# VitalyVorobyev/calibration

Measured on AMD Instinct MI355X. Metric: residual+Jacobian evals/sec, higher is better.
Workload: dtype f64

## Files before the change

calibration_amd/capi.py:

```python
from __future__ import annotations

import ctypes as C
import os
from typing import Optional

import numpy as np

_HERE = os.path.dirname(os.path.abspath(__file__))

CBA_OK, CBA_ERR_INVALID_ARGUMENT, CBA_ERR_RUNTIME, CBA_ERR_NO_DEVICE, CBA_ERR_HIP, CBA_ERR_INTERNAL = range(6)
CHAIN_INTRINSIC, CHAIN_EXTRINSIC, CHAIN_BUNDLE = 0, 1, 2
HANDEYE_DLT, HANDEYE_GIVEN, HANDEYE_TOO_FEW_VIEWS, HANDEYE_NO_PAIRS, HANDEYE_SINGULAR = range(5)
TARGET_ESTIMATED, TARGET_CONFIG, TARGET_IDENTITY = range(3)
LINEAR_OK, LINEAR_TOO_FEW, LINEAR_DEGENERATE = range(3)
LINEAR_MAX_ITERATIONS = 65536
CAMERA_PINHOLE_BC, CAMERA_SCHEIMPFLUG = 0, 1
DTYPE_U8, DTYPE_F32 = 0, 1
IMAGE_MAX_SIDE = 32768
TRI_OK, TRI_NOT_CONVERGED, TRI_BEHIND, TRI_DEGENERATE, TRI_TOO_FEW = range(5)
TRI_MAX_CAMS = 16
TERM_CONVERGENCE, TERM_NO_CONVERGENCE, TERM_FAILURE = 0, 1, 2
RCCL_UNIQUE_ID_BYTES = 128

c_double_p = C.POINTER(C.c_double)
# ... 187 lines not shown

ALLREDUCE_FN = C.CFUNCTYPE(C.c_int32, c_double_p, C.c_int64, C.c_void_p)


class CbaError(RuntimeError):
    def __init__(self, status: int, message: str):
        super().__init__(f"libcalibba status {status}: {message}")
        self.status = status
        self.message = message


class CbaInvalidArgument(CbaError, ValueError):
    """Maps the reference's std::invalid_argument."""


def dptr(a: Optional[np.ndarray]):
    if a is None:
        return C.cast(None, c_double_p)
    assert a.dtype == np.float64 and a.flags["C_CONTIGUOUS"]
    return a.ctypes.data_as(c_double_p)


def i32ptr(a: Optional[np.ndarray]):
    if a is None:
        return C.cast(None, c_int32_p)
    assert a.dtype == np.int32 and a.flags["C_CONTIGUOUS"]
    return a.ctypes.data_as(c_int32_p)


def u8ptr(a: Optional[np.ndarray]):
    if a is None:
        return C.cast(None, c_uint8_p)
    assert a.dtype == np.uint8 and a.flags["C_CONTIGUOUS"]
    return a.ctypes.data_as(c_uint8_p)


def i64ptr(a: Optional[np.ndarray]):
    if a is None:
        return C.cast(None, c_int64_p)
    assert a.dtype == np.int64 and a.flags["C_CONTIGUOUS"]
    return a.ctypes.data_as(c_int64_p)


def library_path() -> str:
    return os.environ.get("CALIBBA_LIBRARY", os.path.join(_HERE, "lib", "libcalibba.so"))


_LIB = None

PROTOTYPES = {
    "cba_version": (C.c_char_p, []),
    "cba_last_error": (C.c_char_p, []),
    "cba_device_count": (C.c_int32, []),
    "cba_trim_cache": (None, []),
    "cba_set_device": (C.c_int32, [C.c_int32]),
    "cba_get_device": (C.c_int32, []),
    "cba_options_default": (None, [C.POINTER(CbaOptions)]),
    "cba_intrinsics_size": (C.c_int32, [C.c_int32]),
    "cba_local_columns": (C.c_int32, [C.c_int32, C.c_int32]),
    "cba_pose_from_matrix": (None, [c_double_p, c_double_p]),
    "cba_pose_to_matrix": (None, [c_double_p, c_double_p]),
    "cba_reproj_create": (C.c_int32, [C.POINTER(CbaReprojProblem), C.c_int32, C.POINTER(C.c_void_p)]),
    "cba_reproj_create_aos": (C.c_int32, [C.POINTER(CbaReprojProblem), C.POINTER(c_double_p), C.c_int32, C.POINTER(C.c_void_p)]),
    "cba_reproj_destroy": (None, [C.c_void_p]),
    "cba_reproj_set_params": (C.c_int32, [C.c_void_p, c_double_p, c_double_p, c_double_p, c_double_p]),
    "cba_reproj_get_params": (C.c_int32, [C.c_void_p, c_double_p, c_double_p, c_double_p, c_double_p]),
    "cba_reproj_num_observations": (C.c_int64, [C.c_void_p]),
    "cba_reproj_eval": (C.c_int32, [C.c_void_p]),
    "cba_reproj_eval_fetch": (C.c_int32, [C.c_void_p, c_double_p, c_double_p]),
    "cba_reproj_eval_fetch_blocks": (C.c_int32, [C.c_void_p, C.c_int32, C.c_int32, c_double_p, c_double_p]),
    "cba_reproj_eval_timed": (C.c_int32, [C.c_void_p, C.c_int32, C.c_int32, c_double_p]),
    "cba_reproj_normal_eq_timed": (C.c_int32, [C.c_void_p, C.c_int32, C.c_int32, c_double_p]),
    "cba_reproj_set_scalar": (C.c_int32, [C.c_void_p, C.c_int32]),
    "cba_reproj_eval_fetch_f32": (C.c_int32, [C.c_void_p, C.POINTER(C.c_float), C.POINTER(C.c_float)]),
    "cba_reproj_cost": (C.c_int32, [C.c_void_p, C.c_double, c_double_p]),
    "cba_reproj_residual_stats": (C.c_int32, [C.c_void_p, C.c_double, c_double_p, c_double_p]),
    "cba_reproj_residuals_fetch_blocks": (C.c_int32, [C.c_void_p, C.c_int32, C.c_int32, C.c_double, c_double_p, c_uint8_p]),
    "cba_reproj_residual_stats_timed": (C.c_int32, [C.c_void_p, C.c_int32, C.c_int32, c_double_p]),
    "cba_reproj_block_normal_eq": (C.c_int32, [C.c_void_p, c_double_p]),
    "cba_reproj_block_normal_eq_size": (C.c_int64, [C.c_void_p]),
    "cba_reproj_solve": (C.c_int32, [C.c_void_p, C.POINTER(CbaOptions), C.POINTER(CbaSummary)]),
    "cba_reproj_set_lm_mode": (C.c_int32, [C.c_void_p, C.c_int32]),
    "cba_reproj_solve_stats": (C.c_int32, [C.c_void_p, C.POINTER(C.c_int64)]),
    "cba_reproj_covariance_dim": (C.c_int64, [C.c_void_p]),
    "cba_reproj_covariance": (C.c_int32, [C.c_void_p, C.POINTER(CbaOptions), c_double_p]),
    "cba_reproj_covariance_shared_dim": (C.c_int64, [C.c_void_p]),
    "cba_reproj_covariance_shared": (C.c_int32, [C.c_void_p, C.POINTER(CbaOptions), c_double_p]),
    "cba_reproj_covariance_views": (C.c_int32, [C.c_void_p, C.POINTER(CbaOptions), C.c_int32, c_int32_p, c_double_p]),
    "cba_reproj_set_allreduce": (C.c_int32, [C.c_void_p, ALLREDUCE_FN, C.c_void_p, C.c_int32, C.c_int32]),
    "cba_rccl_unique_id": (C.c_int32, [C.POINTER(C.c_uint8)]),
    "cba_reproj_init_rccl": (C.c_int32, [C.c_void_p, C.POINTER(C.c_uint8), C.c_int32, C.c_int32]),
    "cba_optimize_intrinsics": (
        C.c_int32,
        [C.c_int32, C.c_int32, c_int64_p, c_double_p, c_double_p, c_double_p, c_double_p, c_double_p, c_double_p,
         C.POINTER(CbaOptions), C.POINTER(CbaSummary), c_double_p],
    ),
    "cba_optimize_extrinsics": (
        C.c_int32,
        [C.c_int32, C.c_int32, C.c_int32, C.c_int32, c_int64_p, c_int32_p, c_int32_p, c_double_p, c_double_p,
         c_double_p, c_double_p, c_double_p, c_double_p, c_double_p, C.POINTER(CbaOptions), C.POINTER(CbaSummary),
         c_double_p],
    ),
    "cba_optimize_bundle": (
        C.c_int32,
        [C.c_int32, C.c_int32, C.c_int32, c_int64_p, c_int32_p, c_double_p, c_double_p, c_double_p, c_double_p,
         c_double_p, c_double_p, c_double_p, c_double_p, C.POINTER(CbaOptions), C.POINTER(CbaSummary), c_double_p],
    ),
    "cba_optimize_planar_pose": (
        C.c_int32,
        [C.c_int32, c_double_p, c_double_p, c_double_p, c_double_p, c_double_p, C.c_int32, c_double_p, C.POINTER(CbaOptions),
         C.POINTER(CbaSummary), c_double_p, c_double_p, c_double_p],
    ),
    "cba_optimize_planar_pose_batch": (
        C.c_int32,
        [C.c_int32, c_int64_p, c_double_p, c_double_p, c_double_p, c_double_p, c_double_p, C.c_int32, c_double_p,
         C.POINTER(CbaOptions), C.POINTER(CbaSummary), c_double_p, c_double_p, c_double_p],
    ),
    "cba_optimize_homography": (
        C.c_int32,
        [C.c_int32, c_double_p, c_double_p, c_double_p, c_double_p, c_double_p, C.POINTER(CbaOptions), C.POINTER(CbaSummary),
         c_double_p],
    ),
    "cba_optimize_homography_batch": (
        C.c_int32,
        [C.c_int32, c_int64_p, c_double_p, c_double_p, c_double_p, c_double_p, c_double_p, C.POINTER(CbaOptions),
         C.POINTER(CbaSummary), c_double_p],
    ),
    "cba_optimize_intrinsics_semidlt": (
        C.c_int32,
        [C.c_int32, c_int64_p, c_double_p, c_double_p, c_double_p, c_double_p, c_double_p, c_double_p, C.c_int32, c_double_p, c_double_p,
         c_int32_p, c_double_p, C.c_int32, C.POINTER(CbaOptions), C.POINTER(CbaSummary), c_double_p, c_double_p, c_double_p],
    ),
    "cba_optimize_intrinsics_semidlt_sharded": (
        C.c_int32,
        [C.c_int32, c_int64_p, c_double_p, c_double_p, c_double_p, c_double_p, C.c_int32, C.c_int32, c_double_p, c_double_p, C.c_int32,
         c_double_p, c_double_p, c_int32_p, c_double_p, C.c_int32, C.POINTER(CbaOptions), C.POINTER(CbaSummary), c_double_p, c_double_p,
         c_double_p, ALLREDUCE_FN, C.c_void_p, C.c_int32, C.c_int32, C.c_int32],
    ),
    "cba_optimize_intrinsics_semidlt_rccl": (
        C.c_int32,
        [C.c_int32, c_int64_p, c_double_p, c_double_p, c_double_p, c_double_p, C.c_int32, C.c_int32, c_double_p, c_double_p, C.c_int32,
         c_double_p, c_double_p, c_int32_p, c_double_p, C.c_int32, C.POINTER(CbaOptions), C.POINTER(CbaSummary), c_double_p, c_double_p,
         c_double_p, C.POINTER(C.c_uint8), C.c_int32, C.c_int32, C.c_int32],
    ),
    "cba_estimate_homography_batch": (
        C.c_int32, [C.c_int32, c_int64_p, c_double_p, c_double_p, c_double_p, c_double_p, c_double_p, c_int32_p]),
    "cba_estimate_planar_pose_batch": (
        C.c_int32, [C.c_int32, c_int64_p, c_double_p, c_double_p, c_double_p, c_double_p, c_double_p, c_double_p]),
    "cba_estimate_handeye_dlt": (C.c_int32, [C.c_int32, c_double_p, c_double_p, C.c_double, c_double_p]),
    "cba_estimate_and_optimize_handeye": (
        C.c_int32,
        [C.c_int32, c_double_p, c_double_p, C.c_double, c_double_p, C.POINTER(CbaOptions), C.POINTER(CbaSummary), c_double_p],
    ),
    "cba_estimate_and_optimize_handeye_sharded": (
        C.c_int32, [C.c_int32, c_double_p, c_double_p, C.c_double, C.c_int32, c_double_p, C.POINTER(CbaOptions), C.POINTER(CbaSummary),
                    c_double_p, ALLREDUCE_FN, C.c_void_p, C.c_int32, C.c_int32, C.c_int32]),
    "cba_estimate_and_optimize_handeye_rccl": (
        C.c_int32, [C.c_int32, c_double_p, c_double_p, C.c_double, C.c_int32, c_double_p, C.POINTER(CbaOptions), C.POINTER(CbaSummary),
                    c_double_p, C.POINTER(C.c_uint8), C.c_int32, C.c_int32, C.c_int32]),
    "cba_optimize_handeye": (
        C.c_int32,
        [C.c_int32, c_double_p, c_double_p, c_double_p, C.POINTER(CbaOptions), C.POINTER(CbaSummary), c_double_p],
    ),
    "cba_plane_fit_options_default": (None, [C.POINTER(CbaPlaneFitOptions)]),
    "cba_calibrate_laser_plane": (
        C.c_int32,
# ... 134 lines not shown
```

calibration_amd/csrc/backend_hip.hip:

```cpp
#include <rccl/rccl.h>

#include <atomic>
#include <cstring>
#include <mutex>
#include <thread>
#include <set>

#include "engine.hpp"
#include "pipelines.hpp"
#include "lm_core.hpp"
#include "lm_state.hpp"
#include "lm_kernels.hpp"

namespace cba {


static inline unsigned nblk(int64_t n, int per) { return static_cast<unsigned>(std::max<int64_t>(1, (n + per - 1) / per)); }

template <class F>
struct ScopeExit {
    F f;
    ~ScopeExit() { f(); }
};
template <class F>
// ... 49 lines not shown
    template <class F>
    void run_stage(HipLMState::GraphSlot& slot, double huber, bool constrained, F&& enqueue) {
        if (!st.graphs_ok) { enqueue(); return; }
        if (slot.huber != huber || slot.constrained != static_cast<int>(constrained) || slot.scalar != e.scalar) {
            if (slot.exec) (void)hipGraphExecDestroy(slot.exec);
            slot.exec = nullptr;
            slot.uses = 0;
            slot.huber = huber; slot.constrained = static_cast<int>(constrained); slot.scalar = e.scalar;
        }
        if (!slot.exec && slot.uses < st.graph_after) {
            ++slot.uses;
            enqueue();
            return;
        }
        if (!slot.exec) {
            if (hipStreamBeginCapture(e.stream, hipStreamCaptureModeThreadLocal) != hipSuccess) {
                (void)hipGetLastError();
                st.graphs_ok = false;
                enqueue();
                return;
            }
            hipGraph_t graph = nullptr;
            try {
                enqueue();
            } catch (...) {
                (void)hipStreamEndCapture(e.stream, &graph);
                if (graph) (void)hipGraphDestroy(graph);
                throw;
            }
            const hipError_t ec = hipStreamEndCapture(e.stream, &graph);
            const hipError_t ei = (ec == hipSuccess && graph) ? hipGraphInstantiate(&slot.exec, graph, nullptr, nullptr, 0) : hipErrorUnknown;
            if (graph) (void)hipGraphDestroy(graph);
            if (ei != hipSuccess) {
                (void)hipGetLastError();
                slot.exec = nullptr;
                st.graphs_ok = false;
                enqueue();
                return;
            }
        }
        CBA_HIP(hipGraphLaunch(slot.exec, e.stream));
    }

    bool prep_normal_eq(std::vector<double>& cam_acc, double cost2[2]) {
        const Structure& s = st.s;
        cam_acc.assign(static_cast<size_t>(s.n_cams) * s.NACC, 0.0);
        cost2[0] = cost2[1] = 0.0;
        return s.n_blocks != 0;
    }
    void enqueue_normal_eq(double huber, int which = 0, double* cam_out = nullptr, double* cost_out = nullptr) {
        enqueue_normal_eq_head(which, huber);
        enqueue_normal_eq_tail(huber, cam_out, cost_out);
    }
    void enqueue_normal_eq_head(int which, double huber = -1.0, bool consts_done = false) {
        if (!consts_done) launch_block_consts(e, which);
        e.head_huber = st.fuse_small ? huber : -1.0;
        ScopeExit reset{[this] { e.head_huber = -1.0; }};
        launch_normal_eq(e);
    }
    void enqueue_normal_eq_tail(double huber, double* cam_out = nullptr, double* cost_out = nullptr) {
        const Structure& s = st.s;
        const size_t nca = static_cast<size_t>(s.n_cams) * s.NACC;
        if (!cam_out) cam_out = st.pin_ne.p;
        if (!cost_out) cost_out = st.pin_ne.p + nca;
        const bool fused_cost = s.n_blocks <= 4096 && !e.head_weights;
        if (e.head_weights)
            ;
        else if (fused_cost)
            hipLaunchKernelGGL(k_weights_cost, dim3(1), dim3(256), 0, e.stream, s.n_blocks, s.NACC, s.NH + s.PL, e.blk_acc.p, huber,
                               e.blk_w.p, e.blk_s.p, cost_out);
        else
            hipLaunchKernelGGL(k_weights, dim3(nblk(s.n_blocks, 256)), dim3(256), 0, e.stream, s.n_blocks, s.NACC, s.NH + s.PL,
                               e.blk_acc.p, huber, e.blk_w.p, e.blk_s.p);
        hipLaunchKernelGGL(k_cam_partial, dim3(std::max(1, st.n_cchunks)), dim3(256), 0, e.stream, s.NACC, st.cchunk_off.p,
                           st.cam_blk.p, e.blk_w.p, e.blk_acc.p, st.cam_partial.p);
        hipLaunchKernelGGL(k_seg_sum, dim3(nblk(s.NACC, RS_COLS), s.n_cams), dim3(RS_COLS * RS_GROUPS), 0, e.stream, s.n_cams,
                           s.NACC, st.cam_seg.p, st.cam_partial.p, cam_out);
        if (!fused_cost) launch_cost(e, huber, cost_out);
        CBA_HIP(hipGetLastError());
    }
    bool vstats_pending = false;
    double ctl_huber = 0.0;
    bool can_fuse() const { return st.fuse_small && st.schur_wave && st.s.n_views != 0 && !e.scalar; }
    void enqueue_system(double huber, bool tail, bool has_blocks, bool constrained, int which, const PackLayout& L, int has_stats, int has_cost = -1) {
        const Structure& s = st.s;
        const bool q2 = s.n_views != 0;
        if (!can_fuse()) {
            if (tail) enqueue_normal_eq_tail(huber, pack_target() + L.cam, st.stat_dev.p + 4);
            if (q2) enqueue_schur(constrained, which, st.sys_tiles.p);
            enqueue_pack(L, has_blocks, q2, has_stats, has_cost);
            return;
        }
        const int n = s.nsh;
        const int64_t sw = static_cast<int64_t>(st.n_pairs) * 4096;
        if (tail && !e.head_weights)
            hipLaunchKernelGGL(k_weights, dim3(nblk(s.n_blocks, 256)), dim3(256), 0, e.stream, s.n_blocks, s.NACC, s.NH + s.PL, e.blk_acc.p,
                               huber, e.blk_w.p, e.blk_s.p);
        SysArgs a{};
        a.d = st.dims; a.n_views = s.n_views; a.n_blocks = s.n_blocks; a.nsh = n; a.n_tiles = st.n_tiles; a.n_pairs = st.n_pairs;
        a.n_vchunks = st.n_vchunks; a.n_cams = s.n_cams; a.NACC = s.NACC; a.constrained = constrained ? 1 : 0;
        a.n_cc = tail ? std::max(1, st.n_cchunks) : 0;
        a.n_vb = static_cast<int>(nblk(s.n_views, 4));
        a.n_costp = tail ? (s.n_blocks <= 4096 ? 1 : (s.n_blocks + 2047) / 2048) : 0;
        a.n_seg_x = static_cast<int>(nblk(s.NACC, RS_COLS));
        a.n_seg = tail ? a.n_seg_x * s.n_cams : 0;
        a.n_syrk = st.n_vchunks * st.n_pairs;
        a.has_vstats = vstats_pending ? 1 : 0;
        a.huber = huber;
        a.link_off = st.link_off.p; a.cchunk_off = st.cchunk_off.p; a.cam_seg = st.cam_seg.p;
        a.link_blk = st.link_blk.p; a.cam_blk = st.cam_blk.p; a.view_fixed = e.view_fixed.p; a.view_cam_blk = st.view_cam_blk.p;
        a.blk_acc = e.blk_acc.p; a.blk_w = e.blk_w.p; a.blk_s = e.blk_s.p; a.lmp = lmp_src; a.view = e.view[which].p;
        a.view_scale2 = e.view_scale2.p; a.view_L = e.view_L.p; a.view_y = e.view_y.p; a.view_D = e.view_D.p; a.view_gp = e.view_gp.p;
        a.blk_Z = e.blk_Z.p; a.view_gmax = st.view_gmax.p; a.cam_partial = st.cam_partial.p; a.cam_out = pack_target() + L.cam;
        if (a.n_costp > 1) e.cost_part.ensure(static_cast<size_t>(2 * a.n_costp));
        a.cost_part = e.cost_part.p; a.cost_out = st.stat_dev.p + 4;
        a.syrk_partial = st.syrk_partial.p; a.tiles_tail = st.sys_tiles.p + sw + n; a.view_stats = st.view_stats.p; a.stat_out = st.stat_dev.p;
        hipLaunchKernelGGL(k_sys_stage2, dim3(a.n_cc + a.n_vb + a.n_costp), dim3(256), 0, e.stream, a);
        const unsigned g3 = static_cast<unsigned>(a.n_seg + a.n_syrk + 1 + a.has_vstats + (a.n_costp > 1 ? 1 : 0));
        if (n >= 64 && st.syrk_mfma) hipLaunchKernelGGL(k_sys_stage3<true>, dim3(g3), dim3(256), 0, e.stream, a);
        else hipLaunchKernelGGL(k_sys_stage3<false>, dim3(g3), dim3(256), 0, e.stream, a);
        vstats_pending = false;
        hipLaunchKernelGGL(k_sys_pack, dim3(nblk(sw + n, RS_COLS)), dim3(RS_COLS * RS_GROUPS), 0, e.stream,
                           pack_args(L, has_blocks, true, has_stats, has_cost), static_cast<int64_t>(st.n_vchunks), st.syrk_partial.p,
                           st.sys_tiles.p + sw + n, st.stat_dev.p, pack_target());
        CBA_HIP(hipGetLastError());
    }
    void collect_normal_eq(std::vector<double>& cam_acc, double cost2[2]) {
        std::memcpy(cam_acc.data(), st.pin_ne.p, sizeof(double) * cam_acc.size());
        cost2[0] = st.pin_ne.p[cam_acc.size()];
        cost2[1] = st.pin_ne.p[cam_acc.size() + 1];
        e.active = 0;
    }
    bool prep_schur(double radius, bool init_scale, std::vector<double>& S, std::vector<double>& g, double* gmax_priv, int* nfail) {
        const Structure& s = st.s;
        const int n = s.nsh;
        S.assign(static_cast<size_t>(n) * n, 0.0);
        g.assign(n, 0.0);
        *gmax_priv = 0.0;
        *nfail = 0;
        if (s.n_views == 0) return false;
        set_lmp(radius, init_scale);
        return true;
    }
    void enqueue_schur(bool constrained, int which = 0, double* tiles_out = nullptr) {
        const Structure& s = st.s;
        const int n = s.nsh;
        const int vpw = st.schur_wave ? 4 : 64;
        hipLaunchKernelGGL(st.schur_wave ? k_schur_view_wave : k_schur_view, dim3(nblk(s.n_views, vpw)), dim3(st.schur_wave ? 256 : 64), 0,
                           e.stream, st.dims, s.n_views, st.link_off.p, st.link_blk.p, e.blk_acc.p, e.blk_w.p, e.view_fixed.p, lmp_src,
                           constrained ? 1 : 0, e.view[which].p, e.view_scale2.p, e.view_L.p, e.view_y.p, e.view_D.p, e.view_gp.p, e.blk_Z.p,
                           st.view_gmax.p);
        const int64_t sw = static_cast<int64_t>(st.n_pairs) * 4096;
        hipLaunchKernelGGL(n >= 64 && st.syrk_mfma ? k_schur_syrk_mfma : k_schur_syrk, dim3(st.n_vchunks, st.n_pairs), dim3(256), 0, e.stream,
                           st.dims, s.n_views, n, st.n_tiles, st.view_cam_blk.p, e.blk_Z.p, e.view_y.p, st.syrk_partial.p);
        double* pack = tiles_out ? tiles_out : st.pin.p;
        hipLaunchKernelGGL(k_row_sum, dim3(nblk(sw + n, RS_COLS)), dim3(RS_COLS * RS_GROUPS), 0, e.stream, static_cast<int64_t>(st.n_vchunks),
                           sw + n, st.syrk_partial.p, pack);
        hipLaunchKernelGGL(k_col_reduce, dim3(1), dim3(256), 0, e.stream, s.n_views, 0, st.view_gmax.p, st.view_gmax.p, pack + sw + n);
        CBA_HIP(hipGetLastError());
    }
    void collect_schur(std::vector<double>& S, std::vector<double>& g, double* gmax_priv, int* nfail) {
        const Structure& s = st.s;
        const int n = s.nsh;
        const int64_t sw = static_cast<int64_t>(st.n_pairs) * 4096;
        const double* tiles = st.pin.p;
        const int32_t nf = static_cast<int32_t>(tiles[static_cast<size_t>(sw) + n + 1] + 0.5);
        for (int i = 0; i < n; ++i) g[i] = tiles[static_cast<size_t>(sw) + i];
        *gmax_priv = tiles[static_cast<size_t>(sw) + n];
        *nfail = nf;
        int pair = 0;
        for (int ti = 0; ti < st.n_tiles; ++ti)
            for (int tj = ti; tj < st.n_tiles; ++tj, ++pair) {
                const double* T = &tiles[static_cast<size_t>(pair) * 4096];
                for (int a = 0; a < 64; ++a) {
                    const int i = ti * 64 + a;
                    if (i >= n) break;
                    for (int b = 0; b < 64; ++b) {
                        const int j = tj * 64 + b;
                        if (j >= n) break;
                        S[static_cast<size_t>(i) * n + j] = T[a * 64 + b];
                        S[static_cast<size_t>(j) * n + i] = T[a * 64 + b];
                    }
                }
            }
    }

    void normal_eq(double huber, std::vector<double>& cam_acc, double cost2[2]) override {
        if (!prep_normal_eq(cam_acc, cost2)) return;
        enqueue_normal_eq(huber);
        CBA_HIP(hipStreamSynchronize(e.stream));
        collect_normal_eq(cam_acc, cost2);
    }
    void schur(double radius, bool init_scale, bool constrained, std::vector<double>& S, std::vector<double>& g, double* gmax_priv,
               int* nfail) override {
        if (!prep_schur(radius, init_scale, S, g, gmax_priv, nfail)) return;
        run_stage(st.g_schur, 0.0, constrained, [&] { enqueue_schur(constrained); });
        CBA_HIP(hipStreamSynchronize(e.stream));
        collect_schur(S, g, gmax_priv, nfail);
    }
    void normal_eq_schur(double huber, std::vector<double>& cam_acc, double cost2[2], double radius, bool init_scale, bool constrained,
                         std::vector<double>& S, std::vector<double>& g, double* gmax_priv, int* nfail) override {
        const bool q1 = prep_normal_eq(cam_acc, cost2);
        const bool q2 = prep_schur(radius, init_scale, S, g, gmax_priv, nfail);
        if (!q1 && !q2) return;
        run_stage(st.g_new, huber, constrained, [&] {
            if (q1) enqueue_normal_eq(huber);
            if (q2) enqueue_schur(constrained);
        });
        CBA_HIP(hipStreamSynchronize(e.stream));
        if (q1) collect_normal_eq(cam_acc, cost2);
        if (q2) collect_schur(S, g, gmax_priv, nfail);
    }
    PackArgs pack_args(const PackLayout& L, bool has_blocks, bool has_schur, int has_stats, int has_cost) const {
        const Structure& s = st.s;
        PackArgs a;
        a.off_stats = L.stats; a.off_cam = L.cam; a.off_cost = L.cost; a.off_nfail = L.nfail; a.off_S = L.S; a.off_g = L.g; a.off_gmax = L.gmax;
        a.n = s.nsh; a.n_tiles = st.n_tiles; a.n_ranks = L.n_ranks; a.rank = e.rank; a.n_cam_doubles = s.n_cams * s.NACC;
        a.has_blocks = has_blocks; a.has_schur = has_schur; a.has_stats = has_stats; a.has_cost = has_cost < 0 ? has_blocks : has_cost;
        return a;
    }
    void ensure_pack(const PackLayout& L) {
        if (st.pack_dev.n < static_cast<size_t>(L.size)) {
            st.pack_dev.alloc(static_cast<size_t>(L.size));
            st.pack_dev.zero(e.stream);
            st.sys_tiles.alloc(static_cast<size_t>(st.n_pairs) * 4096 + st.s.nsh + 8);
            st.stat_dev.alloc(8);
            st.stat_dev.zero(e.stream);
        }
        st.pin_packed.reserve(static_cast<size_t>(L.size));
    }
    bool host_transport() const { return !e.rccl_comm && e.allreduce != nullptr; }
    double* pack_target() { return host_transport() ? st.pin_packed.p : st.pack_dev.p; }
    void enqueue_pack(const PackLayout& L, bool has_blocks, bool has_schur, int has_stats, int has_cost = -1) {
        const int64_t work = std::max<int64_t>({static_cast<int64_t>(st.s.nsh) * st.s.nsh, static_cast<int64_t>(st.s.n_cams) * st.s.NACC, L.n_ranks, 1});
        hipLaunchKernelGGL(k_pack, dim3(nblk(work, 256)), dim3(256), 0, e.stream, pack_args(L, has_blocks, has_schur, has_stats, has_cost),
                           st.stat_dev.p, st.sys_tiles.p, pack_target());
        CBA_HIP(hipGetLastError());
    }
    void wait_step() {
        if (!st.sync_spin) { CBA_HIP(hipStreamSynchronize(e.stream)); return; }
        if (!st.step_done) CBA_HIP(hipEventCreateWithFlags(&st.step_done, hipEventDisableTiming));
        CBA_HIP(hipEventRecord(st.step_done, e.stream));
        const auto t0 = std::chrono::steady_clock::now();
        for (int spins = 0;; ++spins) {
            const hipError_t q = hipEventQuery(st.step_done);
            if (q == hipSuccess) return;
            if (q != hipErrorNotReady) CBA_HIP(q);
#if defined(__x86_64__)
            __builtin_ia32_pause();
#endif
            if ((spins & 63) == 63 && std::chrono::steady_clock::now() - t0 > std::chrono::microseconds(300)) break;
        }
        CBA_HIP(hipStreamSynchronize(e.stream));
    }
    void exchange(int64_t off, int64_t count, const AllReduce& ar, double* host_out, bool to_device = false) {
        if (e.rccl_comm) {
            const ncclResult_t r = ncclAllReduce(st.pack_dev.p + off, st.pack_dev.p + off, static_cast<size_t>(count), ncclDouble, ncclSum,
                                                 reinterpret_cast<ncclComm_t>(e.rccl_comm), e.stream);
            if (r != ncclSuccess) throw HipError(std::string("ncclAllReduce: ") + ncclGetErrorString(r));
            ++device_allreduce_calls;
            device_allreduce_doubles += count;
        } else if (host_transport()) {
            wait_step();
            ar(st.pin_packed.p + off, count);
            if (to_device) st.pack_dev.upload(st.pin_packed.p + off, static_cast<size_t>(count), e.stream, static_cast<size_t>(off));
            if (host_out) std::memcpy(host_out + off, st.pin_packed.p + off, sizeof(double) * static_cast<size_t>(count));
            return;
        } else {
            ++device_allreduce_calls;
            device_allreduce_doubles += count;
        }
        if (host_out) {
            st.pack_dev.download(st.pin_packed.p + off, static_cast<size_t>(count), e.stream, static_cast<size_t>(off));
            wait_step();
            std::memcpy(host_out + off, st.pin_packed.p + off, sizeof(double) * static_cast<size_t>(count));
        }
    }
    void sys_new(double huber, double radius, bool init_scale, bool constrained, const PackLayout& L, const AllReduce& ar, int rank,
                 double* pack) override {
        (void)rank;
        const Structure& s = st.s;
        ensure_pack(L);
        const bool q1 = s.n_blocks != 0;
        set_lmp(radius, init_scale);
        ctl_huber = huber;
        if (q1) enqueue_normal_eq_head(0, huber);
        enqueue_system(huber, q1, q1, constrained, 0, L, 0);
        exchange(L.cam, L.size - L.cam, ar, pack);
        e.active = 0;
    }
    void sys_resolve(double radius, bool constrained, const PackLayout& L, const AllReduce& ar, int rank, double* pack) override {
        (void)rank;
        const Structure& s = st.s;
        ensure_pack(L);
        set_lmp(radius, false);
        enqueue_system(0.0, false, s.n_blocks != 0, constrained, 0, L, 0, 0);
        exchange(L.nfail, L.gmax - L.nfail, ar, pack);
    }
    bool sys_step(const double* delta_sh, double huber, double radius_next, bool constrained, const PackLayout& L, const AllReduce& ar,
                  int rank, double* pack) override {
        (void)rank;
// ... 19 lines not shown
        const bool q1 = s.n_blocks != 0, q2 = s.n_views != 0;
        e.shared_pack[1].upload(st.pin_pack[1].p, e.pk_delta, e.stream);
        if (q2)
            hipLaunchKernelGGL(k_scale_step, dim3(nblk(s.n_views, 64)), dim3(64), 0, e.stream, s.n_views, a, e.view_fixed.p, e.view[0].p,
                               st.view_delta.p, e.view[1].p, st.view_stats.p);
        if (q1 && want_slope) {
            with_alt_blocks([&] {
                enqueue_normal_eq(huber, 1, pack_target() + L.cam, st.stat_dev.p + 4);
                if (q2)
                    hipLaunchKernelGGL(k_view_slope, dim3(nblk(s.n_views, 64)), dim3(64), 0, e.stream, st.dims, s.n_views, st.link_off.p,
                                       st.link_blk.p, e.blk_acc.p, e.blk_w.p, e.view_fixed.p, st.view_delta.p, st.view_stats.p);
            });
        } else if (q1) {
            launch_block_consts(e, 1);
            launch_resid(e);
            launch_cost(e, huber, st.stat_dev.p + 4);
        }
        if (q2)
            hipLaunchKernelGGL(k_col_reduce, dim3(1), dim3(256), 0, e.stream, s.n_views, 4, st.view_stats.p, static_cast<const double*>(nullptr),
                               st.stat_dev.p);
        else
            CBA_HIP(hipMemsetAsync(st.stat_dev.p, 0, 4 * sizeof(double), e.stream));
        CBA_HIP(hipGetLastError());
        enqueue_pack(L, q1 && want_slope, false, 2, q1 ? 1 : 0);
        exchange(0, L.size, ar, pack);
        e.active = 1;
    }
    void launch_accept() {
        const int64_t n_shared = static_cast<int64_t>(e.pk_delta), n_view = static_cast<int64_t>(e.h_view.size());
        hipLaunchKernelGGL(k_accept, dim3(nblk(std::max(n_shared, n_view), 256)), dim3(256), 0, e.stream, n_shared, e.shared_pack[1].p,
                           e.shared_pack[0].p, n_view, e.view[1].p, e.view[0].p);
    }
    void accept_step() override {
        launch_accept();
        const int64_t n_acc = static_cast<int64_t>(st.s.n_blocks) * st.s.NACC, n_w = st.s.n_blocks;
        if (n_acc > 0)
            hipLaunchKernelGGL(k_accept_blocks, dim3(nblk(n_acc, 256)), dim3(256), 0, e.stream, n_acc, e.blk_acc_alt.p, e.blk_acc.p, n_w,
                               e.blk_w_alt.p, e.blk_w.p);
        CBA_HIP(hipGetLastError());
        e.active = 1;
    }

    bool ctl_constrained = false;
    int64_t ctl_invocations = 0;
    void ensure_ctl(const PackLayout& L) {
        const Structure& s = st.s;
        const int n = s.nsh;
        const int lda = ctl_lda(n), M8 = ctl_padded(n);
        const bool lds = lm_ctl_fits_lds(n);
        const size_t o_scal = 0, o_lmp = CS_COUNT, o_camc = o_lmp + 8, o_gc = o_camc + static_cast<size_t>(s.n_cams) * s.NACC, o_scale2 = o_gc + n,
                     o_hdiag = o_scale2 + n, o_xs = o_hdiag + n, o_rdiag = o_xs + M8, o_xtmp = o_rdiag + M8, o_Ld = o_xtmp + e.pk_size,
                     o_A = o_Ld + static_cast<size_t>(M8) * CTL_NB, total = o_A + (lds ? 8 : static_cast<size_t>(M8 + 1) * lda);
        if (st.ctl_n != n || st.ctl_buf.n < total) {
            st.ctl_buf.alloc(total);
            st.ctl_buf.zero(e.stream);
            st.ctl_idx.alloc(static_cast<size_t>(3 * std::max(1, n)));
            st.ctl_eff.alloc(static_cast<size_t>(std::max(1, n)));
            {
                std::vector<int32_t> tab(static_cast<size_t>(3 * std::max(1, n)), 0);
                CtlView T{};
                T.chain = s.chain; T.PC = s.PC;
                for (int i = 0; i < n; ++i) ctl_decode(T, i, &tab[static_cast<size_t>(n) + i], &tab[static_cast<size_t>(2 * n) + i]);
                st.ctl_idx.upload(tab.data(), tab.size(), e.stream);
                CBA_HIP(hipStreamSynchronize(e.stream));
            }
            st.ctl_rec.reserve(CTL_REC_FETCH + e.pk_size + static_cast<size_t>(n) + 8);
            st.ctl_n = n;
        }
        CtlView& V = st.ctl_view;
        V.n = n; V.n_cams = s.n_cams; V.PI = s.PI; V.PL = s.PL; V.NH = s.NH; V.NACC = s.NACC; V.PC = s.PC; V.sh_base = s.sh_base;
        V.chain = s.chain; V.n_ranks = L.n_ranks;
        V.off_stats = L.stats; V.off_cam = L.cam; V.off_cost = L.cost; V.off_nfail = L.nfail; V.off_S = L.S; V.off_g = L.g; V.off_gmax = L.gmax;
        V.pk_cam = static_cast<int64_t>(e.pk_cam); V.pk_target = static_cast<int64_t>(e.pk_target); V.pk_delta = static_cast<int64_t>(e.pk_delta);
        double* b = st.ctl_buf.p;
        V.x_cur = e.shared_pack[0].p; V.x_trial = e.shared_pack[1].p; V.x_tmp = b + o_xtmp;
        V.scal = b + o_scal; V.lmp = b + o_lmp; V.camc = b + o_camc; V.gc = b + o_gc; V.scale2 = b + o_scale2; V.hdiag = b + o_hdiag; V.xs = b + o_xs;
        V.rdiag = b + o_rdiag; V.A = b + o_A; V.Ld = b + o_Ld; V.lda = lda; V.okflag = nullptr;
        V.pack = st.pack_dev.p;
        V.eff = st.ctl_eff.p; V.idx = st.ctl_idx.p; V.colcam = st.ctl_idx.p + n; V.collc = st.ctl_idx.p + 2 * n;
        V.active = st.res_active.p; V.cam_var = st.res_cam_var.p;
        V.rec = st.ctl_rec.p;
    }
    void run_ctl(int mode, int flag) {
        launch_lm_ctl(st.ctl_view, mode, flag, e.stream);
        ++ctl_invocations;
        if (st.ctl_event) {
            if (!st.ctl_done) CBA_HIP(hipEventCreateWithFlags(&st.ctl_done, hipEventDisableTiming));
            CBA_HIP(hipEventRecord(st.ctl_done, e.stream));
        }
    }
    bool ctl_begin(const CtlSetup& cs, const PackLayout& L) override {
        if (!st.lm_ctl_mode) return false;
        const Structure& s = st.s;
        ensure_pack(L);
        ensure_ctl(L);
        ensure_alt_blocks();
        CtlView& V = st.ctl_view;
        V.eps = cs.eps; V.max_iterations = cs.max_iterations; V.constrained = cs.constrained; V.line_search = cs.line_search;
        V.speculate = (cs.speculate && !e.scalar) ? 1 : 0;
        V.intr_var = cs.intr_var; V.target_var = cs.target_var;
        ctl_constrained = cs.constrained;
        st.pin_mask.reserve(static_cast<size_t>(s.nsh + s.n_cams));
        for (int i = 0; i < s.nsh; ++i) st.pin_mask.p[i] = (*cs.active)[i];
        for (int c = 0; c < s.n_cams; ++c) st.pin_mask.p[s.nsh + c] = (*cs.cam_var)[c];
        st.res_active.upload(st.pin_mask.p, s.nsh, e.stream);
        st.res_cam_var.upload(st.pin_mask.p + s.nsh, s.n_cams, e.stream);
        double* stage = st.ctl_rec.p + CS_COUNT;
        ctl_reset(stage);
        stage[CS_COUNT] = 1e4; stage[CS_COUNT + 1] = 1.0;
        st.ctl_buf.upload(stage, CS_COUNT + 2, e.stream);
        for (int k = 0; k < CS_COUNT; ++k) st.ctl_rec.p[k] = 0.0;
        double* pk = st.pin_pack[0].p;
        stage_shared(pk, cs.intr, cs.cam, cs.target);
        e.shared_pack[0].upload(pk, e.pk_delta, e.stream);
        e.shared_pack[1].upload(pk, e.pk_delta, e.stream);
        lmp_src = V.lmp;
        ctl_invocations = 0;
        st.current_is_on_device = false;
        return true;
    }
    void ctl_new(double huber, bool first, const PackLayout& L, const AllReduce& ar, int rank) override {
        (void)rank;
        const Structure& s = st.s;
        const bool q1 = s.n_blocks != 0;
        ctl_huber = huber;
        if (q1) enqueue_normal_eq_head(0, huber);
        enqueue_system(huber, q1, q1, ctl_constrained, 0, L, 0);
        exchange(L.cam, L.size - L.cam, ar, nullptr, true);
        run_ctl(CTL_NEW, first ? 1 : 0);
        e.active = 0;
    }
    void ctl_resolve(const PackLayout& L, const AllReduce& ar, int rank) override {
        (void)rank;
        const Structure& s = st.s;
        enqueue_system(0.0, false, s.n_blocks != 0, ctl_constrained, 0, L, 0, 0);
        exchange(L.nfail, L.gmax - L.nfail, ar, nullptr, true);
        run_ctl(CTL_RESOLVED, 0);
    }
    void launch_backsub(const double* gate, double* stat_out) {
        const Structure& s = st.s;
        hipLaunchKernelGGL(st.schur_wave ? k_backsub_wave : k_backsub, st.schur_wave ? dim3(nblk(s.n_views, 4)) : dim3(nblk(s.n_views, 64)),
                           st.schur_wave ? dim3(256) : dim3(64), 0, e.stream, st.dims, s.n_views, st.link_off.p, st.link_blk.p, e.d_blk_cam.p,
                           e.blk_Z.p, e.delta_sh.p, e.view_fixed.p, e.view_L.p, e.view_y.p, e.view_D.p, e.view_gp.p, e.view[0].p,
                           st.view_delta.p, e.view[1].p, st.view_stats.p, gate);
        hipLaunchKernelGGL(k_col_reduce, dim3(1), dim3(256), 0, e.stream, s.n_views, 4, st.view_stats.p, static_cast<const double*>(nullptr),
                           stat_out, gate);
    }
    void enqueue_backsub() { launch_backsub(e.gate, st.stat_dev.p); }
    void step_head_speculative() {
        const Structure& s = st.s;
        const bool q1 = s.n_blocks != 0, q2 = s.n_views != 0;
        const bool fused_head = q1 && q2 && can_fuse() && e.chain != CBA_CHAIN_BUNDLE;
        if (fused_head) {
#define CBA_STEP_HEAD(CH)                                                                                                                  \
    hipLaunchKernelGGL(k_step_head<CH>, dim3(nblk(s.n_views, 4)), dim3(256), 0, e.stream, e.gate, st.dims, s.n_views, st.link_off.p,         \
                       st.link_blk.p, e.d_blk_cam.p, e.blk_Z.p, e.delta_sh.p, e.view_fixed.p, e.view_L.p, e.view_y.p, e.view_D.p,          \
                       e.view_gp.p, e.view[0].p, st.view_delta.p, e.view[1].p, st.view_stats.p, e.cam[1].p, e.bc.p)
            if (e.chain == CBA_CHAIN_INTRINSIC) CBA_STEP_HEAD(CH_INTRINSIC); else CBA_STEP_HEAD(CH_EXTRINSIC);
#undef CBA_STEP_HEAD
            launch_camera_consts(e, 1);
            vstats_pending = true;
        } else if (q2) {
            enqueue_backsub();
        } else {
            CBA_HIP(hipMemsetAsync(st.stat_dev.p, 0, 4 * sizeof(double), e.stream));
        }
        if (q1) with_alt_blocks([&] { enqueue_normal_eq_head(1, ctl_huber, fused_head); });
    }
    void step_tail_enqueue(double huber, bool constrained, const PackLayout& L) {
        const Structure& s = st.s;
        const bool q1 = s.n_blocks != 0;
        with_alt_blocks([&] { enqueue_system(huber, q1, q1, constrained, 1, L, 1); });
    }
    void step_tail_speculative(double huber, const PackLayout& L, const AllReduce& ar) {
        step_tail_enqueue(huber, ctl_constrained, L);
        exchange(0, L.size, ar, nullptr, true);
        run_ctl(CTL_STEP, 1);
        e.active = 1;
    }
    void ctl_step(double huber, bool speculative, const PackLayout& L, const AllReduce& ar, int rank) override {
        (void)rank;
        const Structure& s = st.s;
        const bool q1 = s.n_blocks != 0, q2 = s.n_views != 0;
        ctl_huber = huber;
        if (speculative) {
            step_head_speculative();
            step_tail_speculative(huber, L, ar);
            return;
        }
        if (q2) enqueue_backsub();
        else CBA_HIP(hipMemsetAsync(st.stat_dev.p, 0, 4 * sizeof(double), e.stream));
        if (q1) {
            launch_block_consts(e, 1);
            launch_resid(e);
            launch_cost(e, huber, st.stat_dev.p + 4);
        } else {
            CBA_HIP(hipMemsetAsync(st.stat_dev.p + 4, 0, sizeof(double), e.stream));
        }
        enqueue_pack(L, false, false, 1, 1);
        exchange(L.stats, 6, ar, nullptr, true);
        run_ctl(CTL_STEP, 0);
        e.active = 1;
    }
    bool pre_vstats_pending = false, pre_head_weights = false;
    bool ctl_prelaunch() override {
        if (!st.ctl_prelaunch || e.scalar || !e.modeb_shared || (e.chain != CBA_CHAIN_INTRINSIC && !e.modeb_moments)) return false;
        pre_vstats_pending = vstats_pending;
        pre_head_weights = e.head_weights;
        ctl_accept(true);
        e.gate = st.ctl_view.scal + CS_GO;
        bool queued = false;
        ScopeExit reset{[&] {
            e.gate = nullptr;
            if (!queued) ctl_prelaunch_cancel();
        }};
        step_head_speculative();
        queued = true;
        return true;
    }
    void ctl_prelaunch_cancel() override {
        ctl_accept(true);
        vstats_pending = pre_vstats_pending;
        e.head_weights = pre_head_weights;
    }
    void ctl_step_tail(double huber, const PackLayout& L, const AllReduce& ar, int rank) override {
        (void)rank;
        step_tail_speculative(huber, L, ar);
    }
    void ctl_accept(bool blocks) override {
        std::swap(e.view[0].p, e.view[1].p);
        if (blocks) swap_block_sets();
        for (HipLMState::GraphSlot* g : {&st.g_new, &st.g_schur, &st.g_trial})
            if (g->exec) { (void)hipGraphExecDestroy(g->exec); g->exec = nullptr; g->uses = 0; }
    }
    const double* ctl_wait() override {
        volatile const double* seq = st.ctl_rec.p + CS_SEQ;
        const double want = static_cast<double>(ctl_invocations);
        if (st.sync_spin) {
            const auto t0 = std::chrono::steady_clock::now();
            for (int spins = 0; *seq < want; ++spins) {
#if defined(__x86_64__)
                __builtin_ia32_pause();
#endif
                if ((spins & 255) == 255 && std::chrono::steady_clock::now() - t0 > std::chrono::microseconds(st.ctl_poll_us)) break;
            }
        }
        if (*seq < want) {
            const auto t0 = std::chrono::steady_clock::now();
            for (int naps = 0; *seq < want; ++naps) {
                std::this_thread::sleep_for(std::chrono::microseconds(st.ctl_event ? 0 : 30));
                if (st.ctl_event) {
                    CBA_HIP(hipEventSynchronize(st.ctl_done));
                    break;
                }
                if ((naps & 31) != 31) continue;
                const hipError_t q = hipStreamQuery(e.stream);
                if (q == hipSuccess) break;
                if (q != hipErrorNotReady) CBA_HIP(q);
// ... 3 lines not shown
                const bool late = std::chrono::steady_clock::now() - t0 > std::chrono::seconds(st.rccl_timeout_s);
                if (async != ncclSuccess || late) {
                    rccl_abort(e);
                    throw HipError(late ? "RCCL exchange: no progress within the deadline (a peer rank failed or hung); communicator aborted"
                                        : std::string("RCCL exchange failed on a peer: ") + ncclGetErrorString(async) + "; communicator aborted");
                }
            }
            if (*seq < want) throw HipError("LM controller: the control record did not arrive");
        }
        std::atomic_thread_fence(std::memory_order_acquire);
        return st.ctl_rec.p;
    }
    void ctl_fetch(double* intr, double* cam, double* target, double* delta) override {
        double* stage = st.ctl_rec.p + CTL_REC_FETCH;
        e.shared_pack[0].download(stage, e.pk_delta, e.stream);
        e.shared_pack[1].download(stage + e.pk_delta, static_cast<size_t>(st.s.nsh), e.stream, e.pk_delta);
        CBA_HIP(hipStreamSynchronize(e.stream));
        unstage_shared(stage, intr, cam, target);
        std::memcpy(delta, stage + e.pk_delta, sizeof(double) * static_cast<size_t>(st.s.nsh));
    }
    void ctl_line_search_done(const double* scal) override {
        double* stage = st.ctl_rec.p + CS_COUNT;
        std::memcpy(stage, scal, sizeof(double) * CS_COUNT);
        st.ctl_buf.upload(stage, CS_COUNT, e.stream);
        run_ctl(CTL_LS_DONE, 0);
    }

    void trial(const double* delta_sh, double huber, TrialStats* out) override {
        const Structure& s = st.s;
        *out = TrialStats();
        if (s.n_blocks == 0) return;
        std::memcpy(st.pin_pack[1].p + e.pk_delta, delta_sh, sizeof(double) * s.nsh);
        run_stage(st.g_trial, huber, false, [&] {
            e.shared_pack[1].upload(st.pin_pack[1].p, e.pk_delta + static_cast<size_t>(s.nsh), e.stream);
            if (s.n_views > 0) launch_backsub(nullptr, st.pin_tr.p + 8);
            launch_block_consts(e, 1);
            launch_resid(e);
            launch_cost(e, huber, st.pin_tr.p + 24);
            CBA_HIP(hipGetLastError());
        });
        CBA_HIP(hipStreamSynchronize(e.stream));
        e.active = 1;
        const double* h = st.pin_tr.p;
        const double* c2 = st.pin_tr.p + 24;
        out->step2 = s.n_views > 0 ? h[8] : 0.0;
        out->xnorm2 = s.n_views > 0 ? h[9] : 0.0;
        out->gd = s.n_views > 0 ? h[10] : 0.0;
        out->dHd = s.n_views > 0 ? h[11] : 0.0;
        out->cost = c2[0];
    }
    void accept() override {
        launch_accept();
        CBA_HIP(hipGetLastError());
        st.current_is_on_device = true;
    }
    void download_private(double* view_pose) override {
        if (e.h_view.empty()) return;
        e.view[0].download(view_pose, e.h_view.size(), e.stream);
        CBA_HIP(hipStreamSynchronize(e.stream));
    }
    void download_blocks(std::vector<double>& acc, std::vector<double>& w) override {
        acc.resize(static_cast<size_t>(e.n_blocks) * e.NACC);
        w.resize(e.n_blocks);
        e.blk_acc.download(acc.data(), acc.size(), e.stream);
        e.blk_w.download(w.data(), w.size(), e.stream);
        CBA_HIP(hipStreamSynchronize(e.stream));
    }
};

void destroy_lm_state(Engine& e) {
    delete lm_state(e);
    e.lm_state = nullptr;
}

void init_lm_state(Engine& e, const cba_reproj_problem& d, bool have_records) {
    auto* st = new HipLMState();
    e.lm_state = st;
    build_structure(d, st->s, have_records);
    const Structure& s = st->s;
    st->dims = SchurDims{s.PL, s.NH, s.NACC, s.PSH, s.PC, s.n_cams, s.chain};
    st->n_vchunks = std::max(1, (s.n_views + VCHUNK - 1) / VCHUNK);
    st->n_tiles = (s.nsh + 63) / 64;
    st->n_pairs = st->n_tiles * (st->n_tiles + 1) / 2;
    std::vector<int64_t> coff{0}, cseg(s.n_cams + 1, 0);
    for (int c = 0; c < s.n_cams; ++c) {
        for (int64_t p = s.cam_off[c]; p < s.cam_off[c + 1]; p += CCHUNK) coff.push_back(std::min<int64_t>(p + CCHUNK, s.cam_off[c + 1]));
        cseg[c + 1] = static_cast<int64_t>(coff.size()) - 1;
    }
    st->n_cchunks = static_cast<int>(coff.size()) - 1;
    auto up64 = [&](DevBuf<int64_t>& b, const std::vector<int64_t>& v) { b.alloc(v.size()); b.upload(v.data(), v.size(), e.stream); };
    auto up32 = [&](DevBuf<int32_t>& b, const std::vector<int32_t>& v) { b.alloc(v.size()); b.upload(v.data(), v.size(), e.stream); };
    up64(st->cchunk_off, coff);
    up64(st->cam_seg, cseg);
    up32(st->cam_blk, s.cam_blk);
    up64(st->link_off, s.link_off);
    up32(st->link_blk, s.link_blk);
    up32(st->view_cam_blk, s.view_cam_blk);
    st->cam_partial.alloc(static_cast<size_t>(std::max(1, st->n_cchunks)) * s.NACC);
    const size_t nv = std::max(1, s.n_views);
    st->view_gmax.alloc(nv);
    st->view_delta.alloc(nv * 6);
    st->view_delta.zero(e.stream);
    st->view_stats.alloc(nv * 4);
    st->syrk_partial.alloc(static_cast<size_t>(st->n_vchunks) * (static_cast<size_t>(st->n_pairs) * 4096 + s.nsh));
    st->pin.reserve(static_cast<size_t>(st->n_pairs) * 4096 + s.nsh + 8);
    st->pin_ne.reserve(static_cast<size_t>(s.n_cams) * s.NACC + 2);
    st->pin_tr.reserve(32);
    st->pin_lmp.reserve(2);
    st->pin_pack[0].reserve(e.pk_size);
    st->pin_pack[1].reserve(e.pk_size);
    {
        hipFuncAttributes fa;
        (void)hipFuncGetAttributes(&fa, reinterpret_cast<const void*>(k_schur_view));
        warm_reproj_kernels();
    }
    if (const char* env = std::getenv("CBA_SYRK_MFMA")) st->syrk_mfma = std::atoi(env);
    if (const char* env = cba_exp_env("CBA_SCHUR_WAVE")) st->schur_wave = std::atoi(env);
    if (const char* env = cba_exp_env("CBA_LM_FUSE")) st->fuse_small = std::atoi(env);
    if (const char* env = cba_exp_env("CBA_LM_CTL_EVENT")) st->ctl_event = std::atoi(env);
    if (const char* env = cba_exp_env("CBA_SYNC_SPIN")) st->sync_spin = std::atoi(env);
    if (const char* env = std::getenv("CBA_LM_GRAPH")) {
        const int v = std::atoi(env);
        st->graphs_ok = v != 0;
        st->graph_after = v > 1 ? v : (v == 1 ? 0 : st->graph_after);
    }
    e.blk_w.alloc(std::max(1, s.n_blocks));
    e.cam_acc.alloc(static_cast<size_t>(s.n_cams) * s.NACC);
    e.view_L.alloc(nv * 36);
    e.view_y.alloc(nv * 6);
    e.view_D.alloc(nv * 6);
    e.view_gp.alloc(nv * 6);
    e.view_scale2.alloc(nv * 6);
    e.view_fixed.alloc(nv);
    e.view_fixed.zero(e.stream);
    e.blk_Z.alloc(static_cast<size_t>(std::max(1, s.n_blocks)) * 6 * s.PSH);
    e.blk_Z.zero(e.stream);
    up64(st->cam_off, s.cam_off);
    st->res_active.alloc(std::max(1, s.nsh));
    st->res_cam_var.alloc(std::max(1, s.n_cams));
    st->res_Hcc.alloc(static_cast<size_t>(s.nsh) * s.nsh);
    st->res_Ssch.alloc(static_cast<size_t>(s.nsh) * s.nsh);
    st->res_out.alloc(32);
    if (const char* env = cba_exp_env("CBA_LM_CTL")) st->lm_ctl_mode = std::atoi(env) != 0;
    if (const char* env = cba_exp_env("CBA_LM_CTL_POLL_US")) st->ctl_poll_us = std::atoi(env);
    if (const char* env = cba_exp_env("CBA_LM_PRELAUNCH")) st->ctl_prelaunch = std::atoi(env);
    if (const char* env = std::getenv("CBA_RCCL_TIMEOUT_S")) st->rccl_timeout_s = std::max(1, std::atoi(env));
    warm_lm_ctl();
    if (const char* env = std::getenv("CBA_LM_RESIDENT")) st->resident_mode = std::atoi(env);
    if (const char* env = std::getenv("CBA_LM_RESIDENT_MAX_OBS")) st->resident_max_obs = std::atoll(env);
    CBA_HIP(hipStreamSynchronize(e.stream));
}

void solve_stats(const Engine& e, int64_t stats8[8]) {
    const HipLMState* st = reinterpret_cast<const HipLMState*>(e.lm_state);
    for (int k = 0; k < 8; ++k) stats8[k] = st ? st->xs[k] : 0;
}

void set_lm_mode(Engine& e, int mode) {
    if (mode < 0 || mode > 3)
        throw std::invalid_argument("lm mode: 0 chip-wide kernels, 1 automatic, 2 resident kernel whenever possible, 3 chip-wide kernels with the host-side iteration (diagnosis)");
    lm_state(e)->resident_mode = mode == 3 ? 0 : mode;
    lm_state(e)->lm_ctl_mode = mode == 3 ? 0 : 1;
}


static LMDriver make_driver(Engine& e, HipBackend& be) {
    AllReduce ar = [&e](double* buf, int64_t n) { engine_allreduce(e, buf, n); };
    return LMDriver(lm_state(e)->s, be, e.h_intr, e.h_cam, e.h_view, e.h_target, ar, e.n_ranks, e.rank);
}

void warm_lm(Engine& e) {
    cba_options o{};
    o.max_iterations = 1;
    const bool resident = resident_lm_eligible(e, o);
    {
        static std::mutex mu;
        static std::set<uint32_t> warmed;
        const uint32_t key = (static_cast<uint32_t>(e.device) << 8) | (resident ? 0x80u : 0u) | (e.scalar ? 0x40u : 0u) |
                             (static_cast<uint32_t>(e.chain) << 2) | static_cast<uint32_t>(e.model);
        std::lock_guard<std::mutex> lock(mu);
        if (!warmed.insert(key).second) return;
    }
    if (resident) { resident_lm_warm(e); return; }
    HipBackend be(e, *lm_state(e));
    const Structure& s = lm_state(e)->s;
    if (s.n_blocks == 0) return;
    std::vector<double> cam_acc, S, g, d(std::max(1, s.nsh), 0.0);
    double c2[2], gm = 0.0;
    int nf = 0;
    std::vector<int32_t> fixed(s.n_views, 0);
    be.set_view_fixed(fixed);
    be.upload_shared(0, e.h_intr.data(), e.h_cam.data(), e.h_target.data());
    be.normal_eq_schur(1.0, cam_acc, c2, 1e4, true, false, S, g, &gm, &nf);
    std::vector<double> S2, g2;
    be.schur(1e4, false, false, S2, g2, &gm, &nf);
    be.upload_shared(1, e.h_intr.data(), e.h_cam.data(), e.h_target.data());
    TrialStats ts;
    be.trial(d.data(), 1.0, &ts);
    {
        const PackLayout L(s, 1);
        std::vector<double> pack(static_cast<size_t>(L.size), 0.0);
        const AllReduce none = [](double*, int64_t) {};
        void* comm = e.rccl_comm;
        e.rccl_comm = nullptr;
        be.sys_new(1.0, 1e4, true, false, L, none, 0, pack.data());
        be.sys_resolve(1e4, false, L, none, 0, pack.data());
        be.upload_shared(1, e.h_intr.data(), e.h_cam.data(), e.h_target.data());
        (void)be.sys_step(d.data(), 1.0, 1e4, false, L, none, 0, pack.data());
        hipLaunchKernelGGL(k_accept_blocks, dim3(1), dim3(64), 0, e.stream, static_cast<int64_t>(0), e.blk_acc_alt.p, e.blk_acc.p,
                           static_cast<int64_t>(0), e.blk_w_alt.p, e.blk_w.p);
        be.ensure_ctl(L);
        double* stage = lm_state(e)->ctl_rec.p + CS_COUNT;
        ctl_reset(stage);
        stage[CS_TERM] = 0.0;
        lm_state(e)->ctl_buf.upload(stage, CS_COUNT, e.stream);
        be.run_ctl(CTL_NEW, 0);
        e.rccl_comm = comm;
    }
    lm_state(e)->g_new.uses = lm_state(e)->g_schur.uses = lm_state(e)->g_trial.uses = 0;
    CBA_HIP(hipStreamSynchronize(e.stream));
}

void solve_lm(Engine& e, const cba_options& o, cba_summary* out) {
    if (resident_lm_eligible(e, o)) {
        for (int k = 0; k < 8; ++k) lm_state(e)->xs[k] = 0;
        if (resident_lm_solve(e, o, out)) return;
    }
    HipBackend be(e, *lm_state(e));
    LMDriver drv = make_driver(e, be);
    try {
        drv.solve(o, out);
    } catch (...) {
        e.gate = nullptr;
        rccl_abort(e);
        throw;
    }
    {
        const ExchangeStats& x = drv.exchange_stats();
// ... 36 lines not shown
```

calibration_amd/csrc/capi.cpp:

```cpp
#include <algorithm>
#include <chrono>
#include <cmath>
#include <cstdlib>
#include <mutex>
#include <thread>
#include <cstring>
#include <memory>
#include <unordered_map>
#include <vector>

#include "capi_common.hpp"
#include "engine.hpp"
#include "pipelines.hpp"
#include "structure.hpp"

using namespace cba;

__attribute__((visibility("hidden"))) thread_local std::string g_err;
__attribute__((visibility("hidden"))) std::atomic<int> g_default_device{0};

Engine::~Engine() {
    if (stream) (void)hipStreamSynchronize(stream);
    rccl_destroy(*this);
    destroy_lm_state(*this);
// ... 668 lines not shown
    double t = thr * thr;
    for (int i = 0; i < 8 && std::sqrt(t) > thr; ++i) t = std::nextafter(t, 0.0);
    for (int i = 0; i < 8; ++i) {
        const double n = std::nextafter(t, HUGE_VAL);
        if (!(std::sqrt(n) <= thr)) break;
        t = n;
    }
    return t;
}

cba_status cba_reproj_residual_stats(cba_reproj* h, double threshold_px, double* blk_stats, double* total) {
    return guarded([&] {
        require_device();
        Engine& e = *as_engine(h);
        const double t2 = keep_bound(threshold_px);
        CBA_HIP(hipSetDevice(e.device));
        residual_stats(e, t2, blk_stats, total);
    });
}

cba_status cba_reproj_residuals_fetch_blocks(cba_reproj* h, int32_t b0, int32_t b1, double threshold_px, double* r, uint8_t* keep) {
    return guarded([&] {
        require_device();
        Engine& e = *as_engine(h);
        const double t2 = keep_bound(threshold_px);
        if (b0 < 0 || b1 < b0 || b1 > e.n_blocks) throw std::invalid_argument("block range outside the problem");
        CBA_HIP(hipSetDevice(e.device));
        residuals_fetch_range(e, b0, b1, t2, r, keep);
    });
}

cba_status cba_reproj_residual_stats_timed(cba_reproj* h, int32_t fetch, int32_t iters, double* ms) {
    return guarded([&] {
        require_device();
        Engine& e = *as_engine(h);
        if (iters <= 0 || !ms) throw std::invalid_argument("iters must be positive and ms given");
        CBA_HIP(hipSetDevice(e.device));
        for (int i = -1; i < iters; ++i) {
            CBA_HIP(hipEventRecord(e.ev0, e.stream));
            if (fetch) residuals_fetch_range(e, 0, e.n_blocks, HUGE_VAL, nullptr, nullptr);
            else residual_stats_launch(e, HUGE_VAL);
            CBA_HIP(hipEventRecord(e.ev1, e.stream));
            CBA_HIP(hipEventSynchronize(e.ev1));
            float t = 0.f;
            CBA_HIP(hipEventElapsedTime(&t, e.ev0, e.ev1));
            if (i >= 0) ms[i] = static_cast<double>(t);
        }
    });
}

int64_t cba_reproj_block_normal_eq_size(const cba_reproj* h) { return h ? reinterpret_cast<const Engine*>(h)->NACC : 0; }

cba_status cba_reproj_block_normal_eq(cba_reproj* h, double* out) {
    return guarded([&] {
        Engine& e = *as_engine(h);
        CBA_HIP(hipSetDevice(e.device));
        launch_block_consts(e, 0);
        launch_normal_eq(e);
        e.blk_acc.download(out, static_cast<size_t>(e.n_blocks) * e.NACC, e.stream);
        CBA_HIP(hipStreamSynchronize(e.stream));
    });
}

cba_status cba_reproj_solve(cba_reproj* h, const cba_options* opts, cba_summary* summary) {
    return guarded([&] {
        Engine& e = *as_engine(h);
        if (!opts || !summary) throw std::invalid_argument("null argument");
        CBA_HIP(hipSetDevice(e.device));
        solve_lm(e, *opts, summary);
    });
}

cba_status cba_reproj_set_lm_mode(cba_reproj* h, int32_t mode) {
    return guarded([&] { set_lm_mode(*as_engine(h), mode); });
}

cba_status cba_reproj_solve_stats(const cba_reproj* h, int64_t stats8[8]) {
    return guarded([&] {
        if (!h || !stats8) throw std::invalid_argument("null argument");
        solve_stats(*reinterpret_cast<const Engine*>(h), stats8);
    });
}

int64_t cba_reproj_covariance_dim(const cba_reproj* h) { return h ? covariance_dim(*reinterpret_cast<const Engine*>(h)) : 0; }

cba_status cba_reproj_covariance(cba_reproj* h, const cba_options* opts, double* cov) {
    return guarded([&] {
        Engine& e = *as_engine(h);
        if (!opts || !cov) throw std::invalid_argument("null argument");
        CBA_HIP(hipSetDevice(e.device));
        compute_covariance(e, *opts, cov);
    });
}

int64_t cba_reproj_covariance_shared_dim(const cba_reproj* h) { return h ? shared_covariance_dim(*reinterpret_cast<const Engine*>(h)) : 0; }

cba_status cba_reproj_covariance_shared(cba_reproj* h, const cba_options* opts, double* cov) {
    return guarded([&] {
        Engine& e = *as_engine(h);
        if (!opts || !cov) throw std::invalid_argument("null argument");
        CBA_HIP(hipSetDevice(e.device));
        compute_covariance(e, *opts, cov, true);
    });
}

cba_status cba_reproj_covariance_views(cba_reproj* h, const cba_options* opts, int32_t n_sel, const int32_t* view_idx, double* cov7x7) {
    return guarded([&] {
        Engine& e = *as_engine(h);
        if (!opts || n_sel < 0 || (n_sel > 0 && (!view_idx || !cov7x7))) throw std::invalid_argument("null argument");
        if (e.chain == CBA_CHAIN_BUNDLE) throw std::invalid_argument("the bundle chain has no per-view poses");
        CBA_HIP(hipSetDevice(e.device));
        if (n_sel > 0) compute_covariance_views(e, *opts, view_idx, n_sel, cov7x7);
    });
}

cba_status cba_reproj_set_allreduce(cba_reproj* h, cba_allreduce_fn fn, void* user, int32_t n_ranks, int32_t rank) {
    return guarded([&] {
        Engine& e = *as_engine(h);
        if (n_ranks < 1 || rank < 0 || rank >= n_ranks) throw std::invalid_argument("bad rank / n_ranks");
        e.allreduce = fn;
        e.allreduce_user = user;
        e.n_ranks = n_ranks;
        e.rank = rank;
    });
}

cba_status cba_rccl_unique_id(uint8_t id[CBA_RCCL_UNIQUE_ID_BYTES]) {
    return guarded([&] { rccl_unique_id(id); });
}

cba_status cba_reproj_init_rccl(cba_reproj* h, const uint8_t id[CBA_RCCL_UNIQUE_ID_BYTES], int32_t n_ranks, int32_t rank) {
    return guarded([&] {
        Engine& e = *as_engine(h);
        CBA_HIP(hipSetDevice(e.device));
        rccl_init(e, id, n_ranks, rank);
    });
}

static void one_shot(const cba_reproj_problem& d, const cba_options* opts, cba_summary* summary, double* cov) {
    if (!opts || !summary) throw std::invalid_argument("null argument");
    PhaseTimer pt;
    auto e = std::make_unique<Engine>();
    build_engine(d, default_device(), *e);
    pt.lap("one-shot: handle");
    solve_lm(*e, *opts, summary);
    pt.lap("one-shot: solve");
    if (d.intr) std::memcpy(d.intr, e->h_intr.data(), sizeof(double) * e->h_intr.size());
    if (d.cam_pose && d.chain != CBA_CHAIN_INTRINSIC) std::memcpy(d.cam_pose, e->h_cam.data(), sizeof(double) * e->h_cam.size());
    if (d.view_pose && !e->h_view.empty()) std::memcpy(d.view_pose, e->h_view.data(), sizeof(double) * e->h_view.size());
    if (d.target_pose && d.chain == CBA_CHAIN_BUNDLE) std::memcpy(d.target_pose, e->h_target.data(), sizeof(double) * 7);
    if (cov && opts->compute_covariance) {
        try {
            compute_covariance(*e, *opts, cov);
        } catch (const HipError&) {
            throw;
        } catch (const std::runtime_error&) {
            const int64_t n = covariance_dim(*e);
            std::memset(cov, 0, sizeof(double) * static_cast<size_t>(n * n));
        }
    }
    CBA_HIP(hipStreamSynchronize(e->stream));
    pt.lap("one-shot: covariance");
    e.reset();
    pt.lap("one-shot: release");
}

// ... 262 lines not shown
```

calibration_amd/csrc/engine.hpp:

```cpp
#pragma once
#include "hip_glue.hpp"
#include "eval_layout.hpp"

#include <deque>
#include <vector>

#include "../../include/calibba.h"

namespace cba {

struct Tile {
    int32_t blk;
    int32_t count;
    int64_t start;
    int64_t xy_start;
    int64_t reserved;
};

constexpr int OPL_B = 32;
constexpr int TILE_B = 64 * OPL_B;

struct EvalFill {
    bool valid = false;
    int blocked = -1, PL = 0, chain = -1, model = -1;
// ... 20 lines not shown
    int64_t n_tilesA = 0, n_tilesB = 0;
    int32_t max_tileB = 0;

    std::vector<double> h_intr, h_cam, h_view, h_target;

    DevBuf<double> X, Y, u, v, r, J;
    std::deque<DevBuf<double>> Jseg;
    EvalFill J_fill, Jf_fill;
    std::deque<EvalFill> Jseg_fill;
    int64_t seg_tiles = 0;
    double* eval_tile_ptr(int64_t w, int64_t tile_doubles) {
        return Jseg.empty() ? J.p + w * tile_doubles : Jseg[static_cast<size_t>(w / seg_tiles)].p + (w % seg_tiles) * tile_doubles;
    }
    int scalar = 0;
    DevBuf<float> Xf, Yf, uf, vf, Jf, bcf, sdf, intrf;
    DevBuf<double> bc, sd, aux;
    DevBuf<double> shared_pack[2];
    size_t pk_cam = 0, pk_target = 0, pk_delta = 0, pk_size = 0;
    DevBuf<double> intr[2], cam[2], view[2], target[2];
    int eval_blocked = 1;
    int eval_done = 0, eval_blocked_last = 0;
    int eval_ablate = 0;
    int eval_variant = 1;
    int active = 0;
    const double* gate = nullptr;
    double head_huber = -1.0;
    bool head_weights = false;
    DevBuf<int32_t> d_blk_cam, d_blk_view;
    DevBuf<Tile> tilesA, tilesB;
    DevBuf<int64_t> d_blk_tile_off;
    DevBuf<double> partial, blk_acc, blk_s, scalar_out;
    DevBuf<double> diag_part, diag_blk, diag_tot;
    DevBuf<double> diag_fpart, diag_ru, diag_rv;
    DevBuf<uint8_t> diag_keep;
    DevBuf<double> cost_part;
    DevBuf<double> blk_mom;
    int modeb_moments = 1;
    int modeb_shared = 1;
    int modeb_split = -1;

    DevBuf<double> blk_w;
    DevBuf<double> blk_acc_alt, blk_w_alt;
    DevBuf<double> cam_acc;
    DevBuf<double> view_L;
    DevBuf<double> view_y;
    DevBuf<double> view_D;
    DevBuf<double> view_gp;
    DevBuf<double> view_scale2;
    DevBuf<double> blk_Z;
    DevBuf<int32_t> view_fixed;
    DevBuf<double> delta_sh;

    cba_allreduce_fn allreduce = nullptr;
    void* allreduce_user = nullptr;
    void* rccl_comm = nullptr;
    int n_ranks = 1, rank = 0;
    DevBuf<double> coll_buf;
    PinnedBuf<double> coll_pin;
    void* lm_state = nullptr;

    ~Engine();
};

void ensure_f32_buffers(Engine& e);
void launch_block_consts(Engine& e, int which);
void launch_camera_consts(Engine& e, int which);
void launch_eval_fill(Engine& e);
void launch_eval(Engine& e);
void launch_resid(Engine& e);
void warm_reproj_kernels();
void launch_normal_eq(Engine& e);
bool launch_normal_eq_shared_rows(Engine& e, double* rows);
void launch_cost(Engine& e, double huber_delta, double* out = nullptr);

void residual_stats_launch(Engine& e, double t2);
void residual_stats(Engine& e, double t2, double* blk_stats, double* total);
void residuals_fetch_range(Engine& e, int b0, int b1, double t2, double* r, uint8_t* keep);

void init_lm_state(Engine& e, const cba_reproj_problem& d, bool have_records = false);
void destroy_lm_state(Engine& e);
void warm_lm(Engine& e);
void solve_lm(Engine& e, const cba_options& o, cba_summary* out);
void solve_stats(const Engine& e, int64_t stats8[8]);
void set_lm_mode(Engine& e, int mode);
void compute_covariance(Engine& e, const cba_options& o, double* cov, bool shared_only = false);
void compute_covariance_views(Engine& e, const cba_options& o, const int32_t* views, int n_sel, double* view_cov);
int64_t covariance_dim(const Engine& e);
int64_t shared_covariance_dim(const Engine& e);
void engine_allreduce(Engine& e, double* host_buf, int64_t count);
void rccl_unique_id(uint8_t* id);
void rccl_init(Engine& e, const uint8_t* id, int n_ranks, int rank);
void rccl_destroy(Engine& e);
void rccl_abort(Engine& e);

}
```

calibration_amd/csrc/lm_core.hpp:

```cpp
#pragma once
#include <algorithm>
#include <chrono>
#include <cmath>
#include <cstdio>
#include <cstdlib>
#include <cstring>
#include <functional>
#include <limits>
#include <stdexcept>
#include <vector>

#include "dense.hpp"
#include "exp_env.hpp"
#include "line_search.hpp"
#include "lm_ctl.hpp"
#include "reproj_math.hpp"
#include "schur_math.hpp"
#include "structure.hpp"

namespace cba {

struct TrialStats {
    double gd = 0, dHd = 0;
    double step2 = 0, xnorm2 = 0;
// ... 205 lines not shown
        double t_wait = 0, t_queue = 0;
        int n_waits = 0, n_head_queued = 0;
        double rec[CS_COUNT];
        auto wait = [&] {
            const auto a = now();
            const double* r = be_.ctl_wait();
            std::memcpy(rec, r, sizeof(rec));
            t_wait += us(a, now());
            ++n_waits;
        };
        be_.ctl_new(huber, true, L_, ar_, rank_);
        wait();
        double last_printed = 0;
        bool pre = false;
        while (rec[CS_TERM] < 0.0) {
            const auto q0 = now();
            const int expect = static_cast<int>(rec[CS_EXPECT]);
            if (o.verbose && rec[CS_P_ITER] > last_printed) {
                last_printed = rec[CS_P_ITER];
                std::printf("[cba] it %3d cost %.12e cand %.12e rel %.3e radius %.3e |g| %.3e%s\n", static_cast<int>(rec[CS_P_ITER]),
                            rec[CS_P_COST], rec[CS_CAND_COST], rec[CS_REL], rec[CS_P_RADIUS], rec[CS_P_GMAX],
                            rec[CS_SPECULATED] != 0.0 ? " (speculative)" : "");
            }
            bool queued_spec = false;
            if (pre && rec[CS_GO] != 0.0) {
                ++n_head_queued;
                be_.ctl_step_tail(huber, L_, ar_, rank_);
                queued_spec = true;
            } else {
                if (pre) be_.ctl_prelaunch_cancel();
                if (rec[CS_ACCEPT] != 0.0) be_.ctl_accept(rec[CS_ACCEPT] == 2.0);
                if (expect == CTL_STEP) {
                    be_.ctl_step(huber, rec[CS_STEP_SPEC] != 0.0, L_, ar_, rank_);
                    queued_spec = rec[CS_STEP_SPEC] != 0.0;
                } else if (expect == CTL_RESOLVED) {
                    be_.ctl_resolve(L_, ar_, rank_);
                    if (pipeline_ && rec[CS_WILL_END] == 0.0) {
                        be_.ctl_step(huber, rec[CS_STEP_SPEC] != 0.0, L_, ar_, rank_);
                        queued_spec = rec[CS_STEP_SPEC] != 0.0;
                    }
                } else if (expect == CTL_NEW) {
                    be_.ctl_new(huber, false, L_, ar_, rank_);
                } else if (expect == CTL_LINE_SEARCH) {
                    ctl_line_search(huber, rec);
                } else {
                    throw std::runtime_error("LM controller: unexpected request");
                }
            }
            pre = prelaunch_ && queued_spec && be_.ctl_prelaunch();
            t_queue += us(q0, now());
            wait();
        }
        if (pre) be_.ctl_prelaunch_cancel();
        if (rec[CS_ACCEPT] != 0.0) be_.ctl_accept(rec[CS_ACCEPT] == 2.0);
        {
            std::vector<double> d(std::max(1, s_.nsh));
            be_.ctl_fetch(intr_.data(), cam_.data(), target_.data(), d.data());
        }
        if (!view_.empty()) be_.download_private(view_.data());
        xs_.allreduce_calls += be_.device_allreduce_calls;
        xs_.allreduce_doubles += be_.device_allreduce_doubles;
        be_.device_allreduce_calls = be_.device_allreduce_doubles = 0;
        xs_.speculative_steps = static_cast<int32_t>(rec[CS_N_SPEC]);
        xs_.speculation_hits = static_cast<int32_t>(rec[CS_N_HITS]);
        xs_.speculation_misses = static_cast<int32_t>(rec[CS_N_MISSES]);
        xs_.rejected_steps = static_cast<int32_t>(rec[CS_N_REJECTED]);
        cost_ = rec[CS_COST];
        const int term = static_cast<int>(rec[CS_TERM]), iter = static_cast<int>(rec[CS_ITER]);
        out->termination = term;
        out->success = term == CBA_TERM_CONVERGENCE;
        out->iterations = iter;
        out->successful_steps = static_cast<int>(rec[CS_SUCCESSFUL]);
        out->initial_cost = rec[CS_INITIAL_COST];
        out->final_cost = cost_;
        out->solve_seconds = std::chrono::duration<double>(std::chrono::steady_clock::now() - t0).count();
        if (timing)
            std::fprintf(stderr, "[cba timing] solve %.1f us, %d iterations, %d waits: waiting %.1f us, host between a wait and the end of its "
                         "launches %.1f us (%.1f per wait; the host computes nothing there: it reads the record and queues launches), %d of the "
                         "waits returned with the next step's head already queued behind the controller (chip idle for the host: 0), "
                         "controller invocations out of turn %d\n", out->solve_seconds * 1e6, iter, n_waits, t_wait, t_queue,
                         t_queue / std::max(1, n_waits), n_head_queued, static_cast<int>(rec[CS_N_WASTED]));
        if (timing && rec[CS_PROF + CP_PUBLISH] > 0.0) {
            static const char* const names[CTL_NPROF] = {"entry", "adopt", "gradient norm", "assemble", "factorise", "back-substitute", "plus",
                                                         "model terms", "decide", "publish", "", ""};
            std::fprintf(stderr, "[cba timing] controller kernel phases, us over %d invocations:", static_cast<int>(rec[CS_SEQ]));
            for (int k = 0; k <= CP_PUBLISH; ++k) std::fprintf(stderr, " %s %.1f |", names[k], rec[CS_PROF + k] * 0.01);
            std::fprintf(stderr, "\n");
        }
        std::snprintf(out->report, sizeof(out->report), "calibba(schur LM, %d rank%s): %s iters=%d cost %.6e -> %.6e", n_ranks_,
                      n_ranks_ > 1 ? "s" : "", ctl_message(static_cast<int>(rec[CS_MSG])), iter, out->initial_cost, cost_);
        return true;
    }

    void ctl_line_search(double huber, const double* rec) {
        const int n = s_.nsh;
        ++xs_.line_searches;
        std::vector<double> full(n), scaled(n), tintr, tcam, ttarget;
        be_.ctl_fetch(intr_.data(), cam_.data(), target_.data(), full.data());
        const double cost0 = rec[CS_COST], slope0 = rec[CS_SLOPE0], dmax = rec[CS_DMAX];
        double step2_sh = 0, xnorm2_sh = 0;
        auto sample = [&](double a, bool with_slope) {
            for (int i = 0; i < n; ++i) scaled[i] = a * full[i];
            shared_plus(scaled, tintr, tcam, ttarget, &step2_sh, &xnorm2_sh);
            be_.upload_shared(1, tintr.data(), tcam.data(), ttarget.data());
            be_.line_eval(a, huber, with_slope, L_, ar_, rank_, pack_.data());
            LineSample ls;
            ls.step = a;
            ls.value = pack_[L_.stats + PackLayout::TRIAL_COST];
            ls.has_value = std::isfinite(ls.value);
            if (with_slope && ls.has_value) {
                const std::vector<double> cam_acc(pack_.begin() + L_.cam, pack_.begin() + L_.cost);
                std::vector<double> Ht(static_cast<size_t>(n) * n), gt(n);
                assemble_shared(cam_acc, Ht, gt);
                double sl = pack_[L_.stats + PackLayout::SLOPE];
                for (int i = 0; i < n; ++i) sl += gt[i] * full[i];
                ls.slope = sl;
                ls.has_slope = std::isfinite(sl);
            }
            return ls;
        };
        int evals = 0;
        LineSample first;
        first.step = 1.0; first.value = rec[CS_CAND_COST]; first.has_value = std::isfinite(first.value);
        double a = armijo_line_search(cost0, slope0, dmax, sample, &evals, &first);
        xs_.line_search_evaluations += evals;
        if (!(a > 0.0)) {
            a = 1.0;
            (void)sample(1.0, false);
            ++xs_.line_search_evaluations;
        }
        double scal[CS_COUNT];
        std::memcpy(scal, rec, sizeof(scal));
        scal[CS_LS_A] = a;
        scal[CS_LS_COST] = pack_[L_.stats + PackLayout::TRIAL_COST];
        scal[CS_LS_STEP2] = pack_[L_.stats + PackLayout::STEP2];
        scal[CS_LS_XNORM2] = pack_[L_.stats + PackLayout::XNORM2];
        scal[CS_LS_STEP2_SH] = step2_sh;
        scal[CS_LS_XNORM2_SH] = xnorm2_sh;
        scal[CS_EXPECT] = CTL_LS_DONE;
        be_.ctl_line_search_done(scal);
    }

    void solve_host(const cba_options& o, cba_summary* out) {
        const auto t0 = std::chrono::steady_clock::now();
        setup(o);
        const int n = s_.nsh;
        const double eps = o.epsilon, huber = o.huber_delta;
        const double min_radius = 1e-32, max_radius = 1e16, min_rel_decrease = 1e-3;
        double radius = 1e4, decrease_factor = 2.0;
        int iter = 0, invalid = 0, successful = 0;

        project_shared();
        xs_ = ExchangeStats();
        be_.upload_shared(0, intr_.data(), cam_.data(), target_.data());
        new_system(radius, true, huber);
        const double initial_cost = cost_;
        int term = CBA_TERM_FAILURE;
        const char* msg = "";
        std::vector<double> delta(n, 0.0), tintr, tcam, ttarget;
        bool plain_next = false;
        double rel_last = 0.0, rel_prev = 0.0;

        auto done = [&](int t, const char* m) { term = t; msg = m; };
        static const bool timing = [] { const char* e = std::getenv("CBA_LM_TIMING"); return e && e[0] == '1'; }();
        double t_reduced = 0, t_step = 0, t_adopt = 0;
        auto now = [] { return std::chrono::steady_clock::now(); };
        auto us = [](std::chrono::steady_clock::time_point a, std::chrono::steady_clock::time_point b) {
            return std::chrono::duration<double, std::micro>(b - a).count();
        };
// ... 575 lines not shown
```

calibration_amd/csrc/lm_ctl.hip:

```cpp
#include <mutex>
#include <set>

#include "engine.hpp"
#include "lm_ctl.hpp"
#include "lm_state.hpp"
#include "wave_reduce.hpp"

namespace cba {

constexpr int CTL_THREADS = 512;
constexpr int CTL_SMALL_N = 136;
constexpr int CTL_WAVES = CTL_THREADS / 64;

struct BlockTeam {
    double* red;
    double* g_scal;
    unsigned long long* last;
    __device__ __forceinline__ int tid() const { return threadIdx.x; }
    __device__ __forceinline__ int size() const { return CTL_THREADS; }
    __device__ __forceinline__ void sync() const { __syncthreads(); }
    __device__ __forceinline__ double sum(double v) const {
        const double t = wave_sum63(v);
        if ((threadIdx.x & 63) == 63) red[threadIdx.x >> 6] = t;
        __syncthreads();
        double s = 0.0;
#pragma unroll
        for (int w = 0; w < CTL_WAVES; ++w) s += red[w];
        __syncthreads();
        return s;
    }
    __device__ __forceinline__ double max(double v) const {
        for (int o = 32; o > 0; o >>= 1) v = fmax(v, __shfl_xor(v, o));
        if ((threadIdx.x & 63) == 0) red[threadIdx.x >> 6] = v;
        __syncthreads();
        double m = red[0];
#pragma unroll
        for (int w = 1; w < CTL_WAVES; ++w) m = fmax(m, red[w]);
        __syncthreads();
        return m;
    }
    __device__ __forceinline__ int count_before(bool flag, int* total) const {
        const unsigned long long mask = __ballot(flag);
        const int lane = threadIdx.x & 63, wave = threadIdx.x >> 6;
        const int before = __popcll(mask & ((1ull << lane) - 1ull));
        if (lane == 0) red[wave] = static_cast<double>(__popcll(mask));
        __syncthreads();
        int base = 0, tot = 0;
#pragma unroll
        for (int w = 0; w < CTL_WAVES; ++w) {
            const int cw = static_cast<int>(red[w]);
            base += w < wave ? cw : 0;
            tot += cw;
        }
        __syncthreads();
        *total = tot;
        return base + before;
    }
    __device__ __forceinline__ void mark(int) const {}
    __device__ __forceinline__ void tick(const CtlView& V, int slot) const {
        if (threadIdx.x == 0) {
            const unsigned long long t = wall_clock64();
            V.scal[CS_PROF + slot] += static_cast<double>(t - *last);
            *last = t;
        }
    }
    __device__ __forceinline__ void publish(const CtlView& V) const {
        tick(V, CP_PUBLISH);
        __syncthreads();
        const int k = threadIdx.x;
        if (k < CS_COUNT) {
            const double v = V.scal[k];
            g_scal[k] = v;
            if (k != CS_SEQ) V.rec[k] = v;
        }
        __threadfence_system();
        __syncthreads();
        if (k == 0) __hip_atomic_store(&V.rec[CS_SEQ], V.scal[CS_SEQ], __ATOMIC_RELEASE, __HIP_MEMORY_SCOPE_SYSTEM);
    }
};

template <bool LDS_A>
__global__ __launch_bounds__(CTL_THREADS) void k_lm_ctl(CtlView V, int mode, int flag) {
    extern __shared__ double lds_dyn[];
    __shared__ double red[CTL_WAVES];
    __shared__ double s_Ld[LDS_A ? CTL_LDS_MAX_N * CTL_NB : 1];
    __shared__ double s_scal[CS_COUNT];
    __shared__ double s_small[5 * CTL_SMALL_N];
    __shared__ int s_idx[3 * CTL_SMALL_N];
    __shared__ int8_t s_flags[3 * CTL_SMALL_N];
    __shared__ int s_ok;
    __shared__ unsigned long long s_last;
    const int tid = threadIdx.x, n = V.n;
    const bool small = LDS_A || n <= CTL_SMALL_N;
    static_assert(CTL_LDS_MAX_N <= CTL_SMALL_N, "the LDS form keeps the short arrays in LDS too");
    double *g_gc = V.gc, *g_scale2 = V.scale2, *g_hdiag = V.hdiag;
    int* g_idx = V.idx;
    int8_t* g_eff = V.eff;
    if (tid < CS_COUNT) s_scal[tid] = V.scal[tid];
    if (tid == 0) s_last = wall_clock64();
    if (small) {
        for (int i = tid; i < n; i += CTL_THREADS) {
            s_small[2 * CTL_SMALL_N + i] = g_gc[i];
            s_small[3 * CTL_SMALL_N + i] = g_scale2[i];
            s_small[4 * CTL_SMALL_N + i] = g_hdiag[i];
            s_idx[i] = g_idx[i];
            s_idx[CTL_SMALL_N + i] = V.colcam[i];
            s_idx[2 * CTL_SMALL_N + i] = V.collc[i];
            s_flags[i] = g_eff[i];
            s_flags[CTL_SMALL_N + i] = V.active[i];
        }
        for (int c = tid; c < V.n_cams && c < CTL_SMALL_N; c += CTL_THREADS) s_flags[2 * CTL_SMALL_N + c] = V.cam_var[c];
        V.rdiag = s_small; V.xs = s_small + CTL_SMALL_N; V.gc = s_small + 2 * CTL_SMALL_N; V.scale2 = s_small + 3 * CTL_SMALL_N;
        V.hdiag = s_small + 4 * CTL_SMALL_N;
        V.idx = s_idx; V.colcam = s_idx + CTL_SMALL_N; V.collc = s_idx + 2 * CTL_SMALL_N;
        V.eff = s_flags; V.active = s_flags + CTL_SMALL_N;
        if (V.n_cams <= CTL_SMALL_N) V.cam_var = s_flags + 2 * CTL_SMALL_N;
    }
    BlockTeam tm{red, V.scal, &s_last};
    V.scal = s_scal;
    V.okflag = &s_ok;
    if (LDS_A) { V.A = lds_dyn; V.Ld = s_Ld; }
    __syncthreads();
    ctl_run(tm, V, mode, flag);
    if (small)
        for (int i = tid; i < n; i += CTL_THREADS) {
            g_gc[i] = s_small[2 * CTL_SMALL_N + i];
            g_scale2[i] = s_small[3 * CTL_SMALL_N + i];
            g_hdiag[i] = s_small[4 * CTL_SMALL_N + i];
            g_idx[i] = s_idx[i];
            g_eff[i] = s_flags[i];
        }
}

size_t lm_ctl_lds_bytes(int n) { return static_cast<size_t>(ctl_padded(n) + 1) * ctl_lda(n) * sizeof(double); }
bool lm_ctl_fits_lds(int n) { return n <= CTL_LDS_MAX_N; }

void launch_lm_ctl(const CtlView& V, int mode, int flag, hipStream_t stream) {
    if (lm_ctl_fits_lds(V.n))
        hipLaunchKernelGGL(k_lm_ctl<true>, dim3(1), dim3(CTL_THREADS), lm_ctl_lds_bytes(V.n), stream, V, mode, flag);
    else
        hipLaunchKernelGGL(k_lm_ctl<false>, dim3(1), dim3(CTL_THREADS), 0, stream, V, mode, flag);
    CBA_HIP(hipGetLastError());
}

void warm_lm_ctl() {
    static std::mutex mu;
    static std::set<int> done;
    int dev = 0;
    CBA_HIP(hipGetDevice(&dev));
    std::lock_guard<std::mutex> lock(mu);
    if (!done.insert(dev).second) return;
    CBA_HIP(hipFuncSetAttribute(reinterpret_cast<const void*>(k_lm_ctl<true>), hipFuncAttributeMaxDynamicSharedMemorySize,
                                static_cast<int>(lm_ctl_lds_bytes(CTL_LDS_MAX_N))));
    hipFuncAttributes fa;
    (void)hipFuncGetAttributes(&fa, reinterpret_cast<const void*>(k_lm_ctl<false>));
}

}
```

calibration_amd/csrc/lm_ctl.hpp:

```cpp
#pragma once
#include <cmath>
#include <cstdint>

#include "../../include/calibba.h"
#include "reproj_math.hpp"
#include "schur_math.hpp"

#if defined(__HIPCC__)
#define CBA_NOINLINE __host__ __device__ __attribute__((noinline))
#else
#define CBA_NOINLINE inline
#endif

namespace cba {

enum CtlSlot : int {
    CS_SEQ = 0,
    CS_TERM,
    CS_MSG,
    CS_EXPECT,
    CS_STEP_SPEC,
    CS_ACCEPT,
    CS_GO,
    CS_WILL_END,
    CS_RADIUS, CS_DECREASE, CS_RADIUS_SPEC, CS_COST, CS_GMAX, CS_GMAX_PRIV, CS_INITIAL_COST, CS_REL_LAST, CS_REL_PREV,
    CS_ITER, CS_SUCCESSFUL, CS_INVALID, CS_VALID, CS_PLAIN_NEXT, CS_NFAIL, CS_M,
    CS_STEP2_SH, CS_XNORM2_SH, CS_GD_SH, CS_DHD_SH, CS_DMAX,
    CS_CAND_COST, CS_REL, CS_MODEL_CHANGE, CS_SLOPE0, CS_SPECULATED,
    CS_P_COST, CS_P_RADIUS, CS_P_GMAX, CS_P_ITER,
    CS_N_SPEC, CS_N_HITS, CS_N_MISSES, CS_N_REJECTED, CS_N_WASTED,
    CS_LS_A, CS_LS_COST, CS_LS_STEP2, CS_LS_XNORM2, CS_LS_STEP2_SH, CS_LS_XNORM2_SH,
    CS_PROF,
    CS_COUNT = 80
};
constexpr int CTL_NPROF = 12;
enum CtlProf : int { CP_ENTRY = 0, CP_ADOPT, CP_GMAX, CP_ASSEMBLE, CP_FACTOR, CP_BACKSOLVE, CP_PLUS, CP_MODEL, CP_DECIDE, CP_PUBLISH };
static_assert(CS_PROF + CTL_NPROF <= CS_COUNT, "control record size");

enum CtlMode : int { CTL_NONE = 0, CTL_NEW = 1, CTL_RESOLVED = 2, CTL_STEP = 3, CTL_LS_DONE = 4, CTL_LINE_SEARCH = 5 };
enum CtlMsg : int { CM_GRADIENT = 0, CM_MAX_ITER, CM_MIN_RADIUS, CM_INVALID_STEPS, CM_PARAMETER, CM_FUNCTION, CM_NONE };
inline const char* ctl_message(int m) {
    static const char* const k[] = {"Gradient tolerance reached.", "Maximum number of iterations reached.",
                                    "Minimum trust region radius reached.", "Number of consecutive invalid steps more than max.",
                                    "Parameter tolerance reached.", "Function tolerance reached.", ""};
    return k[m < 0 || m > CM_NONE ? CM_NONE : m];
}

constexpr int CTL_NB = 8;
CBA_HD int ctl_padded(int n) { return (n + CTL_NB - 1) / CTL_NB * CTL_NB; }
CBA_HD int ctl_lda(int n) { return ctl_padded(n) | 1; }
constexpr int CTL_LDS_MAX_N = 128;

struct CtlView {
    int n, n_cams, PI, PL, NH, NACC, PC, sh_base, chain, n_ranks;
    int64_t off_stats, off_cam, off_cost, off_nfail, off_S, off_g, off_gmax;
    double eps;
    int max_iterations, constrained, line_search, speculate, intr_var, target_var;
    int64_t pk_cam, pk_target, pk_delta;
    double *x_cur, *x_trial, *x_tmp;
    double* scal;
    const double* pack;
    double* camc;
    double *gc, *scale2, *hdiag;
    const int *colcam, *collc;
    int8_t* eff;
    const int8_t *active, *cam_var;
    int* idx;
    double* A;
    int lda;
    double *rdiag, *xs, *Ld;
    int* okflag;
    double* lmp;
    double* rec;
};

struct SerialTeam {
    CBA_HD int tid() const { return 0; }
    CBA_HD int size() const { return 1; }
    CBA_HD void sync() const {}
    CBA_HD double sum(double v) const { return v; }
    CBA_HD double max(double v) const { return v; }
    CBA_HD int count_before(bool flag, int* total) const { *total = flag ? 1 : 0; return 0; }
    CBA_HD void tick(const CtlView&, int) const {}
    CBA_HD void mark(int) const {}
    CBA_HD void publish(const CtlView& V) const {
        for (int k = 1; k < CS_COUNT; ++k) V.rec[k] = V.scal[k];
        V.rec[CS_SEQ] = V.scal[CS_SEQ];
    }
};

CBA_HD bool ctl_finite(double x) { return fabs(x) <= 1.7976931348623157e308; }

CBA_HD void ctl_decode(const CtlView& V, int i, int* cam, int* lc) {
    if (V.chain == CH_BUNDLE) {
        if (i < 6) { *cam = -1; *lc = i; return; }
        *cam = (i - 6) / V.PC;
        *lc = 6 + (i - 6) - *cam * V.PC;
        return;
    }
    *cam = i / V.PC;
    *lc = 6 + i - *cam * V.PC;
}
template <class VW>
CBA_HD int ctl_intr_base(const VW& V, int c) { return V.chain == CH_INTRINSIC ? 0 : V.sh_base + c * V.PC + 6; }
template <class VW>
CBA_HD int ctl_campose_base(const VW& V, int c) { return V.sh_base + c * V.PC; }
CBA_HD int64_t ctl_sidx(int n, int i, int j) { return i <= j ? static_cast<int64_t>(i) * n - static_cast<int64_t>(i) * (i - 1) / 2 + (j - i)
                                                              : static_cast<int64_t>(j) * n - static_cast<int64_t>(j) * (j - 1) / 2 + (i - j); }

struct CtlPlusView {
    int n_cams, PI, PC, sh_base, chain, intr_var, target_var;
    int64_t pk_cam, pk_target;
    const int8_t* cam_var;
};
struct CtlNorms {
    double step2, xnorm2;
};
CBA_HD CtlPlusView ctl_plus_view(const CtlView& V) {
    return CtlPlusView{V.n_cams, V.PI, V.PC, V.sh_base, V.chain, V.intr_var, V.target_var, V.pk_cam, V.pk_target, V.cam_var};
}
template <class TM>
CBA_NOINLINE CtlNorms ctl_plus(TM tm, CtlPlusView V, const double* x, const double* delta, double* xo) {
    double s2 = 0.0, x2 = 0.0;
    const int PI = V.PI;
    for (int i = tm.tid(); i < V.n_cams * PI; i += tm.size()) {
        const int c = i / PI, k = i - c * PI;
        const double p0 = x[i];
        double p = p0;
        if (V.intr_var) {
            p += delta[ctl_intr_base(V, c) + k];
            if (k < 2) p = fmax(p, 0.0);
            s2 += (p - p0) * (p - p0);
            x2 += p0 * p0;
        }
        xo[i] = p;
    }
    if (V.chain != CH_INTRINSIC)
        for (int c = tm.tid(); c < V.n_cams; c += tm.size()) {
            const double* q = x + V.pk_cam + 7 * c;
            double* o = xo + V.pk_cam + 7 * c;
            for (int k = 0; k < 7; ++k) o[k] = q[k];
            if (V.cam_var[c]) {
                const int pb = ctl_campose_base(V, c);
                quat_plus(q, delta + pb, o);
                for (int k = 0; k < 3; ++k) o[4 + k] = q[4 + k] + delta[pb + 3 + k];
                for (int k = 0; k < 7; ++k) { s2 += (o[k] - q[k]) * (o[k] - q[k]); x2 += q[k] * q[k]; }
            }
        }
    if (V.chain == CH_BUNDLE && tm.tid() == tm.size() - 1) {
        const double* q = x + V.pk_target;
        double* o = xo + V.pk_target;
        for (int k = 0; k < 7; ++k) o[k] = q[k];
        if (V.target_var) {
            quat_plus(q, delta, o);
            for (int k = 0; k < 3; ++k) o[4 + k] = q[4 + k] + delta[3 + k];
            for (int k = 0; k < 7; ++k) { s2 += (o[k] - q[k]) * (o[k] - q[k]); x2 += q[k] * q[k]; }
        }
    }
    CtlNorms r;
    r.step2 = tm.sum(s2);
    r.xnorm2 = tm.sum(x2);
    return r;
}

template <class TM>
CBA_HD double ctl_shared_gmax(TM& tm, const CtlView& V) {
    double m = 0.0;
    if (!V.constrained) {
        for (int i = tm.tid(); i < V.n; i += tm.size())
            if (V.eff[i]) m = fmax(m, fabs(V.gc[i]));
        return tm.max(m);
    }
    if (V.chain == CH_INTRINSIC) {
        if (V.intr_var)
            for (int i = tm.tid(); i < V.n_cams * V.PI; i += tm.size()) {
                const int c = i / V.PI, k = i - c * V.PI, col = ctl_intr_base(V, c) + k;
                const double p0 = V.x_cur[i];
                double p = p0 + (V.eff[col] ? -V.gc[col] : 0.0);
                if (k < 2) p = fmax(p, 0.0);
                m = fmax(m, fabs(p - p0));
            }
        return tm.max(m);
    }
    for (int i = tm.tid(); i < V.n; i += tm.size()) V.xs[i] = V.eff[i] ? -V.gc[i] : 0.0;
    tm.sync();
    (void)ctl_plus(tm, ctl_plus_view(V), V.x_cur, V.xs, V.x_tmp);
    for (int i = tm.tid(); i < V.n_cams * V.PI; i += tm.size()) m = fmax(m, fabs(V.x_tmp[i] - V.x_cur[i]));
    if (V.chain != CH_INTRINSIC)
        for (int i = tm.tid(); i < 7 * V.n_cams; i += tm.size()) m = fmax(m, fabs(V.x_tmp[V.pk_cam + i] - V.x_cur[V.pk_cam + i]));
    if (V.chain == CH_BUNDLE)
        for (int i = tm.tid(); i < 7; i += tm.size()) m = fmax(m, fabs(V.x_tmp[V.pk_target + i] - V.x_cur[V.pk_target + i]));
    return tm.max(m);
// ... 365 lines not shown
        gd += V.gc[i] * di;
    }
    {
        const int PL = V.PL, PL2 = PL * PL;
#pragma unroll 4
        for (int e = tm.tid(); e < V.n_cams * PL2; e += tm.size()) {
            const int c = e / PL2, rem = e - c * PL2, li = rem / PL, lj = rem - li * PL;
            const int gi = ctl_shared_col(V, c, li), gj = ctl_shared_col(V, c, lj);
            if (gi < 0 || gj < 0) continue;
            dHd += delta[gi] * V.camc[static_cast<int64_t>(c) * V.NACC + hidx_sym(PL, li, lj)] * delta[gj];
        }
    }
    gd = tm.sum(gd);
    dHd = tm.sum(dHd);
    dmax = tm.max(dmax);
    tm.tick(V, CP_MODEL);
    if (tm.tid() == 0) {
        V.scal[CS_VALID] = 1.0;
        V.scal[CS_STEP2_SH] = s2; V.scal[CS_XNORM2_SH] = x2; V.scal[CS_GD_SH] = gd; V.scal[CS_DHD_SH] = dHd; V.scal[CS_DMAX] = dmax;
        const double rspec = fmin(CTL_MAX_RADIUS, radius / (1.0 / 3.0));
        V.scal[CS_RADIUS_SPEC] = rspec;
        const bool spec = ctl_next_step_speculative(V);
        V.scal[CS_STEP_SPEC] = spec ? 1.0 : 0.0;
        V.scal[CS_EXPECT] = CTL_STEP;
        V.lmp[0] = spec ? rspec : radius;
        V.lmp[1] = 0.0;
    }
}

template <class TM>
CBA_HD bool ctl_decide(TM& tm, const CtlView& V, bool speculated, double model_change, double cand, double step2, double xnorm2) {
    const double eps = V.eps;
    if (tm.tid() == 0) {
        V.scal[CS_INVALID] = 0.0;
        V.scal[CS_P_COST] = V.scal[CS_COST]; V.scal[CS_P_RADIUS] = V.scal[CS_RADIUS]; V.scal[CS_P_GMAX] = V.scal[CS_GMAX];
        V.scal[CS_P_ITER] = V.scal[CS_ITER];
    }
    if (!ctl_finite(cand)) cand = 1.7976931348623157e308;
    const double cost = V.scal[CS_COST];
    const double step_norm = sqrt(step2), x_norm = sqrt(xnorm2);
    const double cost_change = cost - cand;
    const double rel = cost_change / model_change;
    tm.sync();
    if (tm.tid() == 0) { V.scal[CS_CAND_COST] = cand; V.scal[CS_REL] = rel; V.scal[CS_MODEL_CHANGE] = model_change; V.scal[CS_SPECULATED] = speculated ? 1.0 : 0.0; }
    if (step_norm <= eps * (x_norm + eps)) { ctl_end(tm, V, CBA_TERM_CONVERGENCE, CM_PARAMETER); return false; }
    if (fabs(cost_change) <= eps * cost) { ctl_end(tm, V, CBA_TERM_CONVERGENCE, CM_FUNCTION); return false; }
    if (rel > CTL_MIN_REL_DECREASE) {
        for (int64_t i = tm.tid(); i < V.pk_delta; i += tm.size()) V.x_cur[i] = V.x_trial[i];
        const double radius_old = V.scal[CS_RADIUS];
        const double t3 = 2.0 * rel - 1.0;
        const double radius = fmin(CTL_MAX_RADIUS, radius_old / fmax(1.0 / 3.0, 1.0 - t3 * t3 * t3));
        tm.sync();
        if (tm.tid() == 0) {
            V.scal[CS_SUCCESSFUL] += 1.0;
            V.scal[CS_REL_PREV] = V.scal[CS_REL_LAST];
            V.scal[CS_REL_LAST] = fabs(cost_change) / cost;
            V.scal[CS_RADIUS] = radius;
            V.scal[CS_DECREASE] = 2.0;
            V.scal[CS_PLAIN_NEXT] = 0.0;
            V.scal[CS_ACCEPT] = speculated ? 2.0 : 1.0;
            if (!speculated) {
                V.scal[CS_EXPECT] = CTL_NEW;
                V.lmp[0] = radius;
                V.lmp[1] = 0.0;
            }
        }
        tm.sync();
        return speculated;
    }
    if (tm.tid() == 0) {
        V.scal[CS_N_REJECTED] += 1.0;
        const double radius = V.scal[CS_RADIUS] / V.scal[CS_DECREASE];
        V.scal[CS_RADIUS] = radius;
        V.scal[CS_DECREASE] *= 2.0;
        V.scal[CS_PLAIN_NEXT] = 1.0;
        V.scal[CS_EXPECT] = CTL_RESOLVED;
        V.lmp[0] = radius;
        V.lmp[1] = 0.0;
    }
    return false;
}

template <class TM>
CBA_HD void ctl_run(TM& tm, const CtlView& V, int mode, int flag) {
    const bool in_turn = V.scal[CS_TERM] < 0.0 && static_cast<int>(V.scal[CS_EXPECT]) == mode &&
                         (mode != CTL_STEP || (V.scal[CS_STEP_SPEC] != 0.0) == (flag != 0));
    tm.sync();
    if (tm.tid() == 0) {
        V.scal[CS_SEQ] += 1.0;
        V.scal[CS_GO] = 0.0;
        if (in_turn) { V.scal[CS_ACCEPT] = 0.0; V.scal[CS_WILL_END] = 0.0; }
        else V.scal[CS_N_WASTED] += 1.0;
    }
    tm.sync();
    tm.tick(V, CP_ENTRY);
    enum { AFTER_START = 1, AFTER_NEW = 2, AFTER_STEP = 3 };
    int adopt = 0;
    bool iterate = false;
    if (in_turn) {
        if (mode == CTL_NEW) {
            adopt = flag != 0 ? AFTER_START : AFTER_NEW;
        } else if (mode == CTL_RESOLVED) {
            if (tm.tid() == 0) V.scal[CS_NFAIL] = floor(V.pack[V.off_nfail] + 0.5);
            iterate = true;
        } else {
            const double* st = V.pack + V.off_stats;
            const bool speculated = mode == CTL_STEP && flag != 0;
            const double gd = st[0] + V.scal[CS_GD_SH], dHd = st[1] + V.scal[CS_DHD_SH];
            const double model_change = mode == CTL_STEP ? -gd - 0.5 * dHd : V.scal[CS_MODEL_CHANGE];
            const bool valid = model_change > 0.0 && ctl_finite(model_change);
            double cand = st[4], step2 = st[2] + V.scal[CS_STEP2_SH], xnorm2 = st[3] + V.scal[CS_XNORM2_SH];
            if (mode == CTL_LS_DONE) {
                cand = V.scal[CS_LS_COST];
                step2 = V.scal[CS_LS_STEP2] + V.scal[CS_LS_STEP2_SH];
                xnorm2 = V.scal[CS_LS_XNORM2] + V.scal[CS_LS_XNORM2_SH];
            }
            tm.sync();
            if (tm.tid() == 0 && speculated) V.scal[CS_N_SPEC] += 1.0;
            if (!valid) {
                ctl_invalid_step(tm, V);
            } else if (mode == CTL_STEP && V.constrained && V.line_search && !(ctl_finite(cand) && cand <= V.scal[CS_COST] + 1e-4 * gd)) {
                if (tm.tid() == 0) {
                    V.scal[CS_MODEL_CHANGE] = model_change;
                    V.scal[CS_SLOPE0] = gd;
                    V.scal[CS_CAND_COST] = cand;
                    V.scal[CS_EXPECT] = CTL_LINE_SEARCH;
                }
            } else if (ctl_decide(tm, V, speculated, model_change, cand, step2, xnorm2)) {
                adopt = AFTER_STEP;
            }
        }
        tm.sync();
        tm.tick(V, CP_DECIDE);
    }
    if (adopt) {
        ctl_adopt(tm, V, adopt == AFTER_START);
        if (adopt == AFTER_START) {
            if (tm.tid() == 0) V.scal[CS_INITIAL_COST] = V.scal[CS_COST];
            if (V.scal[CS_GMAX] <= V.eps) ctl_end(tm, V, CBA_TERM_CONVERGENCE, CM_GRADIENT);
            else iterate = true;
        } else if (adopt == AFTER_NEW) {
            iterate = true;
        } else if (V.scal[CS_RADIUS] != V.scal[CS_RADIUS_SPEC]) {
            if (tm.tid() == 0) {
                V.scal[CS_N_MISSES] += 1.0;
                V.scal[CS_EXPECT] = CTL_RESOLVED;
                V.lmp[0] = V.scal[CS_RADIUS];
                V.lmp[1] = 0.0;
            }
        } else {
            if (tm.tid() == 0) V.scal[CS_N_HITS] += 1.0;
            iterate = true;
        }
        tm.sync();
    }
    if (iterate) ctl_iterate(tm, V);
    tm.sync();
    if (tm.tid() == 0 && static_cast<int>(V.scal[CS_EXPECT]) == CTL_RESOLVED && V.scal[CS_TERM] < 0.0) {
        int term, msg;
        V.scal[CS_WILL_END] = ctl_top_tests(V, &term, &msg) ? 1.0 : 0.0;
        V.scal[CS_STEP_SPEC] = ctl_next_step_speculative(V) ? 1.0 : 0.0;
    }
    if (tm.tid() == 0)
        V.scal[CS_GO] = (in_turn && V.scal[CS_TERM] < 0.0 && static_cast<int>(V.scal[CS_EXPECT]) == CTL_STEP && V.scal[CS_STEP_SPEC] != 0.0 &&
                         V.scal[CS_ACCEPT] == 2.0) ? 1.0 : 0.0;
    tm.sync();
    tm.publish(V);
// ... 13 lines not shown
```

calibration_amd/csrc/lm_kernels.hpp:

```cpp
#pragma once
#include "block_reduce.hpp"
#include "lm_ctl.hpp"
#include "schur_math.hpp"
#include "wave_reduce.hpp"

namespace cba {

constexpr int VCHUNK = 8;
constexpr size_t CTL_REC_FETCH = 2 * CS_COUNT + 8;
constexpr int CCHUNK = 16;

__global__ void k_weights(int n_blocks, int NACC, int s_idx, const double* __restrict__ blk_acc, double huber_delta,
                          double* __restrict__ blk_w, double* __restrict__ blk_s) {
    const int b = blockIdx.x * blockDim.x + threadIdx.x;
    if (b >= n_blocks) return;
    const double s = blk_acc[static_cast<int64_t>(b) * NACC + s_idx];
    double rho, w;
    huber(s, huber_delta, &rho, &w);
    blk_w[b] = w;
    blk_s[b] = s;
}

__global__ __launch_bounds__(256) void k_weights_cost(int n_blocks, int NACC, int s_idx, const double* __restrict__ blk_acc,
                                                      double huber_delta, double* __restrict__ blk_w, double* __restrict__ blk_s,
                                                      double* __restrict__ out) {
    __shared__ double sh[2][256];
    double c = 0.0, ss = 0.0;
    constexpr int NQ = 16;
    for (int b0 = static_cast<int>(threadIdx.x); b0 < n_blocks; b0 += NQ * 256) {
        double sv[NQ];
#pragma unroll
        for (int q = 0; q < NQ; ++q) {
            const int b = b0 + q * 256;
            sv[q] = b < n_blocks ? blk_acc[static_cast<int64_t>(b) * NACC + s_idx] : 0.0;
        }
#pragma unroll
        for (int q = 0; q < NQ; ++q) {
            const int b = b0 + q * 256;
            if (b < n_blocks) {
                double rho, w;
                huber(sv[q], huber_delta, &rho, &w);
                blk_w[b] = w;
                blk_s[b] = sv[q];
                c += 0.5 * rho;
                ss += sv[q];
            }
        }
    }
    block_sum2(sh, c, ss, out);
}

__device__ __forceinline__ void cam_partial_body(int k, int NACC, const int64_t* __restrict__ chunk_off, const int32_t* __restrict__ cam_blk,
                                                 const double* __restrict__ blk_w, const double* __restrict__ blk_acc,
                                                 double* __restrict__ partial) {
    const int64_t p0 = chunk_off[k], p1 = chunk_off[k + 1];
    for (int e = threadIdx.x; e < NACC; e += blockDim.x) {
        double s = 0.0;
        for (int64_t p = p0; p < p1; p += CCHUNK) {
            double a[CCHUNK], w[CCHUNK];
#pragma unroll
            for (int q = 0; q < CCHUNK; ++q) {
                const bool in = p + q < p1;
                const int b = in ? cam_blk[p + q] : 0;
                w[q] = in ? blk_w[b] : 0.0;
                a[q] = in ? blk_acc[static_cast<int64_t>(b) * NACC + e] : 0.0;
            }
#pragma unroll
            for (int q = 0; q < CCHUNK; ++q)
                if (p + q < p1) s += w[q] * a[q];
        }
        partial[static_cast<int64_t>(k) * NACC + e] = s;
    }
}
__global__ void k_cam_partial(int NACC, const int64_t* __restrict__ chunk_off, const int32_t* __restrict__ cam_blk,
                              const double* __restrict__ blk_w, const double* __restrict__ blk_acc,
                              double* __restrict__ partial) {
    cam_partial_body(blockIdx.x, NACC, chunk_off, cam_blk, blk_w, blk_acc, partial);
}

constexpr int RS_COLS = 32, RS_GROUPS = 8;

__device__ __forceinline__ double grouped_column_sum(const double* __restrict__ rows, int64_t t0, int64_t t1, int64_t width,
                                                     int64_t e, bool valid, double (*sh)[RS_COLS]) {
    const int c = threadIdx.x % RS_COLS, r = threadIdx.x / RS_COLS;
    double s = 0.0;
    if (valid)
// ... 198 lines not shown
    const int c = threadIdx.x;
    if (c >= 64 || c0 + c >= nsh) return;
    double s = 0.0;
    for (int r = 0; r < nrow; ++r) s += Zs[r][c] * ysh[r];
    out[c0 + c] = s;
}

constexpr int SYRK_ROWS = 6 * VCHUNK;
constexpr int SYRK_LDS = 2 * SYRK_ROWS * 64 + SYRK_ROWS + VCHUNK * SYRK_MAX_CAMS / 2;

__device__ __forceinline__ void tile_pair(int pair, int n_tiles, int* ti, int* tj) {
    int i = 0;
    while (pair >= n_tiles - i) { pair -= n_tiles - i; ++i; }
    *ti = i;
    *tj = i + pair;
}

__device__ __forceinline__ void syrk_tile_valu(const double (*Zi)[64], const double (*Zc)[64], int nrow, double* __restrict__ out) {
    const int tx = threadIdx.x & 15, ty = threadIdx.x >> 4;
    double acc[4][4];
#pragma unroll
    for (int a = 0; a < 4; ++a)
#pragma unroll
        for (int b = 0; b < 4; ++b) acc[a][b] = 0.0;
    for (int r = 0; r < nrow; ++r) {
        double a[4], b[4];
#pragma unroll
        for (int q = 0; q < 4; ++q) { a[q] = Zi[r][ty * 4 + q]; b[q] = Zc[r][tx * 4 + q]; }
#pragma unroll
        for (int p = 0; p < 4; ++p)
#pragma unroll
            for (int q = 0; q < 4; ++q) acc[p][q] += a[p] * b[q];
    }
#pragma unroll
    for (int p = 0; p < 4; ++p)
#pragma unroll
        for (int q = 0; q < 4; ++q) out[(ty * 4 + p) * 64 + tx * 4 + q] = acc[p][q];
}

typedef double v4f64 __attribute__((ext_vector_type(4)));
__device__ __forceinline__ void syrk_tile_mfma(const double (*Zi)[64], const double (*Zc)[64], double* __restrict__ out) {
    const int lane = threadIdx.x & 63, wave = threadIdx.x >> 6;
    const int li = lane & 15, lk = lane >> 4;
    v4f64 acc[4];
#pragma unroll
    for (int c = 0; c < 4; ++c) acc[c] = v4f64{0.0, 0.0, 0.0, 0.0};
#pragma unroll
    for (int step = 0; step < SYRK_ROWS / 4; ++step) {
        const int r = 4 * step + lk;
        const double a = Zi[r][wave * 16 + li];
#pragma unroll
        for (int c = 0; c < 4; ++c) acc[c] = __builtin_amdgcn_mfma_f64_16x16x4f64(a, Zc[r][c * 16 + li], acc[c], 0, 0, 0);
    }
#pragma unroll
    for (int c = 0; c < 4; ++c)
#pragma unroll
        for (int reg = 0; reg < 4; ++reg) out[(wave * 16 + lk + 4 * reg) * 64 + c * 16 + li] = acc[c][reg];
}

template <bool MFMA>
__device__ __forceinline__ void schur_syrk_body(double* lds, int bx, int by, int gy, const SchurDims& d, int n_views, int nsh, int n_tiles,
        const int32_t* __restrict__ view_cam_blk, const double* __restrict__ blk_Z, const double* __restrict__ y, double* __restrict__ partial) {
    double (*Zi)[64] = reinterpret_cast<double (*)[64]>(lds), (*Zj)[64] = Zi + SYRK_ROWS;
    double* ysh = lds + 2 * SYRK_ROWS * 64;
    int* bsh = reinterpret_cast<int*>(ysh + SYRK_ROWS);
    int ti, tj;
    tile_pair(by, n_tiles, &ti, &tj);
    const int i0 = ti * 64, j0 = tj * 64;
    const int v0 = bx * VCHUNK;
    const int nrow = 6 * (min(n_views, v0 + VCHUNK) - v0);
    stage_block_table(d, n_views, v0, view_cam_blk, bsh);
    __syncthreads();
    stage_Z(d, bsh, n_views, v0, view_cam_blk, blk_Z, i0, nsh, Zi);
    if (tj != ti) stage_Z(d, bsh, n_views, v0, view_cam_blk, blk_Z, j0, nsh, Zj);
    if (static_cast<int>(threadIdx.x) < SYRK_ROWS) ysh[threadIdx.x] = static_cast<int>(threadIdx.x) < nrow ? y[6 * static_cast<int64_t>(v0) + threadIdx.x] : 0.0;
    __syncthreads();
    const double (*Zc)[64] = tj != ti ? Zj : Zi;
    double* row = partial + static_cast<int64_t>(bx) * (static_cast<int64_t>(gy) * 4096 + nsh);
    double* out = row + static_cast<int64_t>(by) * 4096;
    if constexpr (MFMA) syrk_tile_mfma(Zi, Zc, out);
    else syrk_tile_valu(Zi, Zc, nrow, out);
    if (ti == tj) schur_gvec_chunk(Zi, ysh, nrow, i0, nsh, row + static_cast<int64_t>(gy) * 4096);
}
__global__ __launch_bounds__(256) void k_schur_syrk(SchurDims d, int n_views, int nsh, int n_tiles, const int32_t* __restrict__ view_cam_blk,
        const double* __restrict__ blk_Z, const double* __restrict__ y, double* __restrict__ partial) {
    __shared__ double lds[SYRK_LDS];
    schur_syrk_body<false>(lds, blockIdx.x, blockIdx.y, gridDim.y, d, n_views, nsh, n_tiles, view_cam_blk, blk_Z, y, partial);
}
__global__ __launch_bounds__(256) void k_schur_syrk_mfma(SchurDims d, int n_views, int nsh, int n_tiles, const int32_t* __restrict__ view_cam_blk,
        const double* __restrict__ blk_Z, const double* __restrict__ y, double* __restrict__ partial) {
    __shared__ double lds[SYRK_LDS];
    schur_syrk_body<true>(lds, blockIdx.x, blockIdx.y, gridDim.y, d, n_views, nsh, n_tiles, view_cam_blk, blk_Z, y, partial);
}

__global__ void k_backsub(SchurDims d, int n_views, const int64_t* __restrict__ link_off, const int32_t* __restrict__ link_blk,
                          const int32_t* __restrict__ blk_cam, const double* __restrict__ blk_Z,
                          const double* __restrict__ delta_sh, const int32_t* __restrict__ fixed, const double* __restrict__ L,
                          const double* __restrict__ y, const double* __restrict__ D, const double* __restrict__ gp,
                          const double* __restrict__ x, double* __restrict__ delta_p, double* __restrict__ xt,
                          double* __restrict__ stats , const double* __restrict__ gate = nullptr) {
    if (gate && *gate == 0.0) return;
    const int v = blockIdx.x * blockDim.x + threadIdx.x;
    if (v >= n_views) return;
    const int nb = static_cast<int>(link_off[v + 1] - link_off[v]);
    double o4[4];
    backsub_view_body(d, nb, link_blk + link_off[v], blk_cam, blk_Z, delta_sh, fixed[v] != 0, L + 36 * static_cast<int64_t>(v),
                      y + 6 * static_cast<int64_t>(v), D + 6 * static_cast<int64_t>(v), gp + 6 * static_cast<int64_t>(v),
                      x + 7 * static_cast<int64_t>(v), delta_p + 6 * static_cast<int64_t>(v), xt + 7 * static_cast<int64_t>(v), o4);
    for (int k = 0; k < 4; ++k) stats[4 * static_cast<int64_t>(v) + k] = o4[k];
}

__global__ void k_accept(int64_t n_shared, const double* __restrict__ shared_trial, double* __restrict__ shared_cur, int64_t n_view,
                         const double* __restrict__ view_trial, double* __restrict__ view_cur) {
    const int64_t i = static_cast<int64_t>(blockIdx.x) * blockDim.x + threadIdx.x;
    if (i < n_shared) shared_cur[i] = shared_trial[i];
    if (i < n_view) view_cur[i] = view_trial[i];
}

struct PackArgs {
    int64_t off_stats, off_cam, off_cost, off_nfail, off_S, off_g, off_gmax;
    int n, n_tiles, n_ranks, rank, n_cam_doubles;
    int has_blocks , has_cost , has_schur, has_stats;
};
__device__ __forceinline__ void pack_scalars(const PackArgs& a, const double* __restrict__ stat, double nfail, double* __restrict__ pack) {
    pack[a.off_nfail] = nfail;
    pack[a.off_cost] = a.has_cost ? stat[4] : 0.0;
    pack[a.off_stats + 0] = a.has_stats == 1 ? stat[2] : 0.0;
    pack[a.off_stats + 1] = a.has_stats == 1 ? stat[3] : 0.0;
    pack[a.off_stats + 2] = a.has_stats ? stat[0] : 0.0;
    pack[a.off_stats + 3] = a.has_stats ? stat[1] : 0.0;
    pack[a.off_stats + 4] = (a.has_stats && a.has_cost) ? stat[4] : 0.0;
    pack[a.off_stats + 5] = a.has_stats == 2 ? stat[2] : 0.0;
}
__global__ __launch_bounds__(256) void k_pack(PackArgs a, const double* __restrict__ stat ,
                                              const double* __restrict__ tiles , double* __restrict__ pack) {
    const int64_t tid = static_cast<int64_t>(blockIdx.x) * blockDim.x + threadIdx.x;
    const int64_t nn = static_cast<int64_t>(a.n) * a.n;
    const int64_t sw = static_cast<int64_t>(a.n_tiles) * (a.n_tiles + 1) / 2 * 4096;
    if (tid < nn) {
        const int i = static_cast<int>(tid / a.n), j = static_cast<int>(tid % a.n);
        if (i <= j) {
            double val = 0.0;
            if (a.has_schur) {
                const int ti = i >> 6, tj = j >> 6;
                const int pair = ti * a.n_tiles - ti * (ti - 1) / 2 + (tj - ti);
                val = tiles[static_cast<int64_t>(pair) * 4096 + (i & 63) * 64 + (j & 63)];
            }
            pack[a.off_S + ctl_sidx(a.n, i, j)] = val;
        }
    }
    if (tid < a.n) pack[a.off_g + tid] = a.has_schur ? tiles[sw + tid] : 0.0;
    if (tid < a.n_ranks) pack[a.off_gmax + tid] = (a.has_schur && tid == a.rank) ? tiles[sw + a.n] : 0.0;
    if (tid == 0) pack_scalars(a, stat, a.has_schur ? tiles[sw + a.n + 1] : 0.0, pack);
    if (!a.has_blocks && tid < a.n_cam_doubles) pack[a.off_cam + tid] = 0.0;
}

struct SysArgs {
    SchurDims d;
    int n_views, n_blocks, nsh, n_tiles, n_pairs, n_vchunks, n_cams, NACC, constrained;
    int n_cc, n_vb, n_costp;
    int n_seg_x, n_seg, n_syrk;
    int has_vstats;
    double huber;
    const int64_t *link_off, *cchunk_off, *cam_seg;
    const int32_t *link_blk, *cam_blk, *view_fixed, *view_cam_blk;
    const double *blk_acc, *blk_w, *blk_s, *lmp, *view;
    double *view_scale2, *view_L, *view_y, *view_D, *view_gp, *blk_Z, *view_gmax, *cam_partial, *cam_out, *cost_part, *cost_out;
    double *syrk_partial, *tiles_tail , *view_stats, *stat_out;
};

__global__ __launch_bounds__(256) void k_sys_stage2(SysArgs a) {
    __shared__ double lds[2 * 256];
    int bx = blockIdx.x;
    if (bx < a.n_cc) {
        cam_partial_body(bx, a.NACC, a.cchunk_off, a.cam_blk, a.blk_w, a.blk_acc, a.cam_partial);
        return;
    }
    bx -= a.n_cc;
    if (bx < a.n_vb) {
        schur_view_wave_body(bx, a.d, a.n_views, a.link_off, a.link_blk, a.blk_acc, a.blk_w, a.view_fixed, a.lmp, a.constrained, a.view,
                             a.view_scale2, a.view_L, a.view_y, a.view_D, a.view_gp, a.blk_Z, a.view_gmax);
        return;
    }
    bx -= a.n_vb;
    if (a.n_costp == 1) cost_range_body(lds, 0, a.n_blocks, a.blk_s, a.huber, a.cost_out);
    else cost_range_body(lds, bx * 2048, min(bx * 2048 + 2048, a.n_blocks), a.blk_s, a.huber, a.cost_part + 2 * bx);
}

template <bool MFMA>
__global__ __launch_bounds__(256) void k_sys_stage3(SysArgs a) {
    __shared__ double lds[SYRK_LDS];
    static_assert(SYRK_LDS >= COL_REDUCE_LDS && SYRK_LDS >= RS_GROUPS * RS_COLS, "one LDS buffer for every body");
    int bx = blockIdx.x;
    if (bx < a.n_seg) {
        seg_sum_body(lds, bx % a.n_seg_x, bx / a.n_seg_x, a.NACC, a.cam_seg, a.cam_partial, a.cam_out);
        return;
    }
    bx -= a.n_seg;
    if (bx < a.n_syrk) {
        const int chunk = bx % a.n_vchunks, pair = bx / a.n_vchunks;
        schur_syrk_body<MFMA>(lds, chunk, pair, a.n_pairs, a.d, a.n_views, a.nsh, a.n_tiles, a.view_cam_blk, a.blk_Z, a.view_y, a.syrk_partial);
        return;
    }
    bx -= a.n_syrk;
    if (bx == 0) { col_reduce_body(lds, a.n_views, 0, a.view_gmax, a.view_gmax, a.tiles_tail); return; }
    if (bx == 1 && a.has_vstats) { col_reduce_body(lds, a.n_views, 4, a.view_stats, nullptr, a.stat_out); return; }
    if (threadIdx.x == 0) {
        double c = 0.0, ss = 0.0;
        for (int k = 0; k < a.n_costp; ++k) { c += a.cost_part[2 * k]; ss += a.cost_part[2 * k + 1]; }
        a.cost_out[0] = c;
        a.cost_out[1] = ss;
    }
}

__global__ __launch_bounds__(RS_COLS * RS_GROUPS) void k_sys_pack(PackArgs a, int64_t n_rows, const double* __restrict__ rows,
                                                                   const double* __restrict__ tail ,
                                                                   const double* __restrict__ stat, double* __restrict__ pack) {
    __shared__ double sh[RS_GROUPS][RS_COLS];
    const int64_t sw = static_cast<int64_t>(a.n_tiles) * (a.n_tiles + 1) / 2 * 4096, width = sw + a.n;
    const int64_t e = static_cast<int64_t>(blockIdx.x) * RS_COLS + threadIdx.x % RS_COLS;
    const double tot = grouped_column_sum(rows, 0, n_rows, width, e, e < width, sh);
    if (threadIdx.x < RS_COLS && e < width) {
        if (e < sw) {
            int ti, tj;
            tile_pair(static_cast<int>(e >> 12), a.n_tiles, &ti, &tj);
            const int i = ti * 64 + static_cast<int>((e >> 6) & 63), j = tj * 64 + static_cast<int>(e & 63);
            if (i <= j && j < a.n) pack[a.off_S + ctl_sidx(a.n, i, j)] = tot;
        } else {
            pack[a.off_g + (e - sw)] = tot;
        }
    }
    const int64_t tid = static_cast<int64_t>(blockIdx.x) * blockDim.x + threadIdx.x;
    if (tid < a.n_ranks) pack[a.off_gmax + tid] = tid == a.rank ? tail[0] : 0.0;
    if (tid == 0) pack_scalars(a, stat, tail[1], pack);
    if (!a.has_blocks)
        for (int64_t k = tid; k < a.n_cam_doubles; k += static_cast<int64_t>(gridDim.x) * blockDim.x) pack[a.off_cam + k] = 0.0;
}

template <int CHAIN>
__global__ __launch_bounds__(256) void k_step_head(const double* __restrict__ gate, SchurDims d, int n_views, const int64_t* __restrict__ link_off,
                                                   const int32_t* __restrict__ link_blk, const int32_t* __restrict__ blk_cam,
                                                   const double* __restrict__ blk_Z, const double* __restrict__ delta_sh,
                                                   const int32_t* __restrict__ fixed, const double* __restrict__ L, const double* __restrict__ y,
                                                   const double* __restrict__ D, const double* __restrict__ gp, const double* __restrict__ x,
                                                   double* __restrict__ delta_p, double* __restrict__ xt, double* __restrict__ stats,
                                                   const double* __restrict__ cam_trial, double* __restrict__ bc) {
    if (gate && *gate == 0.0) return;
    const int v = blockIdx.x * 4 + (threadIdx.x >> 6), lane = threadIdx.x & 63;
    if (v >= n_views) return;
    const int nb = static_cast<int>(link_off[v + 1] - link_off[v]);
    const int32_t* blks = link_blk + link_off[v];
    const bool fx = fixed[v] != 0;
    double a[6];
    backsub_wave_sums(d, nb, blks, blk_cam, blk_Z, delta_sh, fx, lane, a);
    double pose[7] = {0.0, 0.0, 0.0, 0.0, 0.0, 0.0, 0.0};
    if (lane == 63) {
        double o4[4], dp[6];
        backsub_view_finish(fx, a, L + 36 * static_cast<int64_t>(v), y + 6 * static_cast<int64_t>(v), D + 6 * static_cast<int64_t>(v),
                            gp + 6 * static_cast<int64_t>(v), x + 7 * static_cast<int64_t>(v), dp, pose, o4);
        for (int k = 0; k < 6; ++k) delta_p[6 * static_cast<int64_t>(v) + k] = dp[k];
        for (int k = 0; k < 7; ++k) xt[7 * static_cast<int64_t>(v) + k] = pose[k];
        for (int k = 0; k < 4; ++k) stats[4 * static_cast<int64_t>(v) + k] = o4[k];
    }
#pragma unroll
    for (int k = 0; k < 7; ++k) pose[k] = __shfl(pose[k], 63);
    for (int k = lane; k < nb; k += 64) {
        const int b = blks[k];
        double out[BC_SIZE];
        block_consts<CHAIN>(pose, CHAIN == CH_EXTRINSIC ? cam_trial + 7 * static_cast<int64_t>(blk_cam[b]) : nullptr, nullptr, out);
        for (int i = 0; i < BC_SIZE; ++i) bc[static_cast<int64_t>(b) * BC_SIZE + i] = out[i];
    }
}

__global__ void k_scale_step(int n_views, double a, const int32_t* __restrict__ fixed, const double* __restrict__ x,
                             const double* __restrict__ delta_p, double* __restrict__ xt, double* __restrict__ stats) {
    const int v = blockIdx.x * blockDim.x + threadIdx.x;
    if (v >= n_views) return;
    double o2[2];
    scale_step_view_body(fixed[v] != 0, a, x + 7 * static_cast<int64_t>(v), delta_p + 6 * static_cast<int64_t>(v), xt + 7 * static_cast<int64_t>(v), o2);
    stats[4 * static_cast<int64_t>(v)] = o2[0];
    stats[4 * static_cast<int64_t>(v) + 1] = o2[1];
    stats[4 * static_cast<int64_t>(v) + 2] = 0.0;
    stats[4 * static_cast<int64_t>(v) + 3] = 0.0;
}
__global__ void k_view_slope(SchurDims d, int n_views, const int64_t* __restrict__ link_off, const int32_t* __restrict__ link_blk,
                             const double* __restrict__ blk_acc, const double* __restrict__ blk_w, const int32_t* __restrict__ fixed,
                             const double* __restrict__ delta_p, double* __restrict__ stats) {
    const int v = blockIdx.x * blockDim.x + threadIdx.x;
    if (v >= n_views) return;
    stats[4 * static_cast<int64_t>(v) + 2] = view_slope_body(d, static_cast<int>(link_off[v + 1] - link_off[v]), link_blk + link_off[v], blk_acc,
                                                              blk_w, fixed[v] != 0, delta_p + 6 * static_cast<int64_t>(v));
}

__global__ void k_accept_blocks(int64_t n_acc, const double* __restrict__ acc_trial, double* __restrict__ acc_cur, int64_t n_w,
                                const double* __restrict__ w_trial, double* __restrict__ w_cur) {
    const int64_t i = static_cast<int64_t>(blockIdx.x) * blockDim.x + threadIdx.x;
    if (i < n_acc) acc_cur[i] = acc_trial[i];
    if (i < n_w) w_cur[i] = w_trial[i];
}

}
```

calibration_amd/csrc/lm_state.hpp:

```cpp
#pragma once
#include "engine.hpp"
#include "lm_ctl.hpp"
#include "schur_math.hpp"
#include "structure.hpp"

namespace cba {

struct HipLMState {
    Structure s;
    SchurDims dims;
    int n_vchunks = 0, n_tiles = 0, n_pairs = 0, n_cchunks = 0;
    int fuse_small = 1;
    int schur_wave = 1;
    int syrk_mfma = 1;
    DevBuf<int32_t> view_cam_blk, cam_blk;
    DevBuf<int64_t> cchunk_off, cam_seg, link_off;
    DevBuf<int32_t> link_blk;
    DevBuf<double> cam_partial, view_gmax, view_delta, view_stats, syrk_partial;
    PinnedBuf<double> pin, pin_ne, pin_tr;
    DevBuf<double> pack_dev, sys_tiles, stat_dev;
    PinnedBuf<double> pin_packed;
    hipEvent_t step_done = nullptr;
    hipEvent_t ctl_done = nullptr;
    int ctl_event = 0;
    int sync_spin = 1;
    ~HipLMState() {
        if (step_done) (void)hipEventDestroy(step_done);
        if (ctl_done) (void)hipEventDestroy(ctl_done);
    }
    int64_t xs[8] = {0, 0, 0, 0, 0, 0, 0, 0};
    struct GraphSlot {
        hipGraphExec_t exec = nullptr;
        double huber = 0.0;
        int constrained = -1, scalar = -1;
        int uses = 0;
        ~GraphSlot() { if (exec) (void)hipGraphExecDestroy(exec); }
    };
    GraphSlot g_new, g_schur, g_trial;
    bool graphs_ok = true;
    int graph_after = 200;
    PinnedBuf<double> pin_lmp;
    PinnedBuf<double> pin_pack[2];
    bool current_is_on_device = false;
    int resident_mode = 1;
    int64_t resident_max_obs = -1;
    DevBuf<int64_t> cam_off;
    DevBuf<int8_t> res_active, res_cam_var;
    DevBuf<double> res_Hcc, res_Ssch, res_out;
    PinnedBuf<double> pin_res;
    PinnedBuf<int8_t> pin_mask;
    DevBuf<double> ctl_buf;
    DevBuf<int32_t> ctl_idx;
    DevBuf<int8_t> ctl_eff;
    PinnedBuf<double> ctl_rec;
    CtlView ctl_view{};
    int ctl_n = -1;
    int rccl_timeout_s = 120;
    int ctl_prelaunch = 1;
    int ctl_poll_us = 2000;
    int lm_ctl_mode = 1;
};


inline HipLMState* lm_state(Engine& e) { return reinterpret_cast<HipLMState*>(e.lm_state); }

bool resident_lm_eligible(const Engine& e, const cba_options& o);
void resident_lm_warm(Engine& e);
bool resident_lm_solve(Engine& e, const cba_options& o, cba_summary* out, bool keep_parameters = false);

void launch_lm_ctl(const CtlView& V, int mode, int flag, hipStream_t stream);
bool lm_ctl_fits_lds(int n);
void warm_lm_ctl();

}
```

calibration_amd/optim.py:

```python
from __future__ import annotations

import ctypes as C
from dataclasses import dataclass, field
from typing import List, Optional, Sequence

import numpy as np

from . import capi
from .capi import CbaOptions, CbaReprojProblem, CbaSummary, dptr, i32ptr, i64ptr


@dataclass
class OptimOptions:
    optimizer: int = 0
    huber_delta: float = 1.0
    epsilon: float = 1e-9
    max_iterations: int = 1000
    compute_covariance: bool = True
    verbose: bool = False


@dataclass
class OptimResult:
    success: bool = False
# ... 287 lines not shown
                getattr(f, name)[...] = np.asarray(val, dtype=np.float64).reshape(getattr(f, name).shape)
        capi.check(self.lib, self.lib.cba_reproj_set_params(self.h, dptr(f.intr), dptr(f.cam_pose), dptr(f.view_pose),
                                                            dptr(f.target_pose)))

    def get_params(self):
        f = self.flat
        capi.check(self.lib, self.lib.cba_reproj_get_params(self.h, dptr(f.intr), dptr(f.cam_pose), dptr(f.view_pose),
                                                            dptr(f.target_pose)))
        return f.intr, f.cam_pose, f.view_pose, f.target_pose

    def eval(self):
        capi.check(self.lib, self.lib.cba_reproj_eval(self.h))

    def eval_fetch(self):
        n, p = self.n_obs, self.local_columns
        r = np.zeros(2 * n)
        J = np.zeros((2 * n, p))
        capi.check(self.lib, self.lib.cba_reproj_eval_fetch(self.h, dptr(r), dptr(J)))
        return r, J

    def eval_fetch_blocks(self, b0: int, b1: int):
        n, p = int(self.flat.blk_offset[b1] - self.flat.blk_offset[b0]), self.local_columns
        r = np.zeros(2 * n)
        J = np.zeros((2 * n, p))
        capi.check(self.lib, self.lib.cba_reproj_eval_fetch_blocks(self.h, int(b0), int(b1), dptr(r), dptr(J)))
        return r, J

    def set_scalar(self, scalar: int):
        capi.check(self.lib, self.lib.cba_reproj_set_scalar(self.h, int(scalar)))

    def eval_fetch_f32(self):
        n, p = self.n_obs, self.local_columns
        r = np.zeros(2 * n, dtype=np.float32)
        J = np.zeros((2 * n, p), dtype=np.float32)
        capi.check(self.lib, self.lib.cba_reproj_eval_fetch_f32(self.h, r.ctypes.data_as(C.POINTER(C.c_float)),
                                                                J.ctypes.data_as(C.POINTER(C.c_float))))
        return r, J

    def eval_timed(self, warmup: int, iters: int) -> float:
        ms = C.c_double(0.0)
        capi.check(self.lib, self.lib.cba_reproj_eval_timed(self.h, int(warmup), int(iters), C.byref(ms)))
        return float(ms.value)

    def normal_eq_timed(self, warmup: int, iters: int) -> float:
        ms = C.c_double()
        capi.check(self.lib, self.lib.cba_reproj_normal_eq_timed(self.h, int(warmup), int(iters), C.byref(ms)))
        return ms.value

    def cost(self, huber_delta: float = 1.0) -> float:
        c = C.c_double(0.0)
        capi.check(self.lib, self.lib.cba_reproj_cost(self.h, float(huber_delta), C.byref(c)))
        return float(c.value)

    def residual_stats(self, threshold_px: float = float("inf")):
        from .diagnostics import ResidualStats

        nb = self.flat.n_blocks
        blk = np.zeros((max(nb, 1), 4))
        tot = np.zeros(4)
        capi.check(self.lib, self.lib.cba_reproj_residual_stats(self.h, float(threshold_px), dptr(blk), dptr(tot)))
        return ResidualStats.from_flat(self.flat, blk[:nb], tot, float(threshold_px))

    def residuals_fetch_blocks(self, b0: int, b1: int, threshold_px: float = float("inf")):
        n = int(self.flat.blk_offset[b1] - self.flat.blk_offset[b0]) if 0 <= b0 <= b1 <= self.flat.n_blocks else 0
        r = np.zeros(max(2 * n, 1))
        keep = np.zeros(max(n, 1), dtype=np.uint8)
        capi.check(self.lib, self.lib.cba_reproj_residuals_fetch_blocks(self.h, int(b0), int(b1), float(threshold_px), dptr(r),
                                                                        capi.u8ptr(keep)))
        return r[:2 * n], keep[:n].astype(bool)

    def residual_stats_timed(self, iters: int = 5, fetch: bool = False) -> np.ndarray:
        ms = np.zeros(int(iters))
        capi.check(self.lib, self.lib.cba_reproj_residual_stats_timed(self.h, int(bool(fetch)), int(iters), dptr(ms)))
        return ms

    def block_normal_eq(self) -> np.ndarray:
        w = int(self.lib.cba_reproj_block_normal_eq_size(self.h))
        out = np.zeros((self.flat.n_blocks, w))
        capi.check(self.lib, self.lib.cba_reproj_block_normal_eq(self.h, dptr(out)))
        return out

    def set_lm_mode(self, mode: int):
        capi.check(self.lib, self.lib.cba_reproj_set_lm_mode(self.h, int(mode)))

    def solve_stats(self) -> dict:
        a = (C.c_int64 * 8)()
        capi.check(self.lib, self.lib.cba_reproj_solve_stats(self.h, a))
        return dict(zip(("allreduce_calls", "allreduce_doubles", "speculative_steps", "speculation_hits", "speculation_misses",
                         "rejected_steps", "line_searches", "line_search_evaluations"), (int(v) for v in a)))

    def solve(self, opts: CbaOptions) -> CbaSummary:
        s = CbaSummary()
        capi.check(self.lib, self.lib.cba_reproj_solve(self.h, C.byref(opts), C.byref(s)))
        self.get_params()
        return s

    def covariance(self, opts: CbaOptions) -> Optional[np.ndarray]:
        dim = int(self.lib.cba_reproj_covariance_dim(self.h))
        cov = np.zeros((dim, dim))
        st = self.lib.cba_reproj_covariance(self.h, C.byref(opts), dptr(cov))
        if st == capi.CBA_ERR_RUNTIME:
            return None
        capi.check(self.lib, st)
        return cov

    def covariance_shared(self, opts: CbaOptions) -> Optional[np.ndarray]:
        n = int(self.lib.cba_reproj_covariance_shared_dim(self.h))
        cov = np.zeros((n, n))
        st = self.lib.cba_reproj_covariance_shared(self.h, C.byref(opts), dptr(cov))
        if st == capi.CBA_ERR_RUNTIME:
            return None
        capi.check(self.lib, st)
        return cov

    def covariance_views(self, opts: CbaOptions, view_idx) -> Optional[np.ndarray]:
        idx = np.ascontiguousarray(view_idx, dtype=np.int32)
        out = np.zeros((len(idx), 7, 7))
        st = self.lib.cba_reproj_covariance_views(self.h, C.byref(opts), len(idx), i32ptr(idx), dptr(out))
        if st == capi.CBA_ERR_RUNTIME:
            return None
        capi.check(self.lib, st)
        return out

    def set_allreduce(self, fn, n_ranks: int, rank: int):

        def _cb(buf, count, _user):
            try:
                arr = np.ctypeslib.as_array(buf, shape=(int(count),))
                fn(arr)
                return 0
            except Exception:
                return 1

        self._cb = capi.ALLREDUCE_FN(_cb)
        capi.check(self.lib, self.lib.cba_reproj_set_allreduce(self.h, self._cb, None, int(n_ranks), int(rank)))

    def init_rccl(self, unique_id: bytes, n_ranks: int, rank: int):
        buf = (C.c_uint8 * capi.RCCL_UNIQUE_ID_BYTES).from_buffer_copy(unique_id)
        capi.check(self.lib, self.lib.cba_reproj_init_rccl(self.h, buf, int(n_ranks), int(rank)))


def rccl_unique_id(lib=None) -> bytes:
    lib = lib or capi.load_library()
    buf = (C.c_uint8 * capi.RCCL_UNIQUE_ID_BYTES)()
    capi.check(lib, lib.cba_rccl_unique_id(buf))
    return bytes(buf)


def _solve_flat(flat: FlatProblem, copts: CbaOptions, device: int = 0):
    with ReprojHandle(flat, device) as h:
        s = h.solve(copts)
        cov = h.covariance(copts) if copts.compute_covariance else None
    return s, cov


def optimize_intrinsics(views, init_camera, init_c_se3_t, opts: Optional[IntrinsicsOptimOptions] = None,
                        device: int = 0) -> IntrinsicsOptimizationResult:
    opts = opts or IntrinsicsOptimOptions()
    if len(views) < 4:
        raise capi.CbaInvalidArgument(capi.CBA_ERR_INVALID_ARGUMENT,
                                      "Insufficient views for calibration (at least 4 required).")
    flat = flatten_intrinsics(views, init_camera, init_c_se3_t)
    s, cov = _solve_flat(flat, to_cba_options(opts.core, True, opts.optimize_skew), device)
    return IntrinsicsOptimizationResult(result_core(s, cov), flat.intr.reshape(-1).copy(),
                                        [pose_to_matrix(p) for p in flat.view_pose.reshape(-1, 7)])

# ... 294 lines not shown
```

include/calibba.h:

```cpp
#ifndef CALIBBA_H
#define CALIBBA_H

#include <stdint.h>

#ifdef __cplusplus
extern "C" {
#endif

#define CBA_VERSION_STRING "0.1.0"

typedef enum cba_status {
    CBA_OK = 0,
    CBA_ERR_INVALID_ARGUMENT = 1,
    CBA_ERR_RUNTIME = 2,
    CBA_ERR_NO_DEVICE = 3,
    CBA_ERR_HIP = 4,
    CBA_ERR_INTERNAL = 5
} cba_status;

typedef enum cba_chain {
    CBA_CHAIN_INTRINSIC = 0,
    CBA_CHAIN_EXTRINSIC = 1,
    CBA_CHAIN_BUNDLE = 2
} cba_chain;
// ... 21 lines not shown

typedef struct cba_summary {
    int32_t success;
    int32_t termination;
    int32_t iterations;
    int32_t successful_steps;
    double initial_cost;
    double final_cost;
    double solve_seconds;
    char report[192];
} cba_summary;

typedef struct cba_reproj_problem {
    int32_t chain;
    int32_t camera_model;
    int32_t n_blocks;
    int32_t n_cams;
    int32_t n_views;
    int32_t reserved0;
    int64_t first_view_global;
    const int64_t* blk_offset;
    const int32_t* blk_cam;
    const int32_t* blk_view;
    const double* blk_b_T_g;
    const double* X;
    const double* Y;
    const double* u;
    const double* v;
    double* intr;
    double* cam_pose;
    double* view_pose;
    double* target_pose;
} cba_reproj_problem;

typedef struct cba_reproj cba_reproj;

const char* cba_version(void);
const char* cba_last_error(void);
int32_t cba_device_count(void);
void cba_trim_cache(void);
cba_status cba_set_device(int32_t device);
int32_t cba_get_device(void);
void cba_options_default(cba_options* o);
int32_t cba_intrinsics_size(int32_t camera_model);
int32_t cba_local_columns(int32_t chain, int32_t camera_model);

void cba_pose_from_matrix(const double* m44_colmajor, double* pose7);
void cba_pose_to_matrix(const double* pose7, double* m44_colmajor);

cba_status cba_reproj_create(const cba_reproj_problem* desc, int32_t device, cba_reproj** out);
cba_status cba_reproj_create_aos(const cba_reproj_problem* desc, const double* const* blk_obs, int32_t device, cba_reproj** out);
void cba_reproj_destroy(cba_reproj* h);
cba_status cba_reproj_set_params(cba_reproj* h, const double* intr, const double* cam_pose,
                                 const double* view_pose, const double* target_pose);
cba_status cba_reproj_get_params(cba_reproj* h, double* intr, double* cam_pose, double* view_pose,
                                 double* target_pose);
int64_t cba_reproj_num_observations(const cba_reproj* h);

cba_status cba_reproj_eval(cba_reproj* h);
cba_status cba_reproj_eval_fetch(cba_reproj* h, double* r, double* J);
cba_status cba_reproj_eval_fetch_blocks(cba_reproj* h, int32_t b0, int32_t b1, double* r, double* J);
cba_status cba_reproj_eval_timed(cba_reproj* h, int32_t warmup, int32_t iters, double* ms_per_eval);

cba_status cba_reproj_normal_eq_timed(cba_reproj* h, int32_t warmup, int32_t iters, double* ms_per_pass);

cba_status cba_reproj_set_scalar(cba_reproj* h, int32_t scalar);
cba_status cba_reproj_eval_fetch_f32(cba_reproj* h, float* r, float* J);

cba_status cba_reproj_cost(cba_reproj* h, double huber_delta, double* cost);

cba_status cba_reproj_residual_stats(cba_reproj* h, double threshold_px, double* blk_stats, double* total);
cba_status cba_reproj_residuals_fetch_blocks(cba_reproj* h, int32_t b0, int32_t b1, double threshold_px, double* r,
                                             uint8_t* keep);
cba_status cba_reproj_residual_stats_timed(cba_reproj* h, int32_t fetch, int32_t iters, double* ms);

cba_status cba_reproj_block_normal_eq(cba_reproj* h, double* out);
int64_t cba_reproj_block_normal_eq_size(const cba_reproj* h);

cba_status cba_reproj_solve(cba_reproj* h, const cba_options* opts, cba_summary* summary);

cba_status cba_reproj_set_lm_mode(cba_reproj* h, int32_t mode);

cba_status cba_reproj_solve_stats(const cba_reproj* h, int64_t stats8[8]);

int64_t cba_reproj_covariance_dim(const cba_reproj* h);
cba_status cba_reproj_covariance(cba_reproj* h, const cba_options* opts, double* cov );

int64_t cba_reproj_covariance_shared_dim(const cba_reproj* h);
cba_status cba_reproj_covariance_shared(cba_reproj* h, const cba_options* opts, double* cov );
cba_status cba_reproj_covariance_views(cba_reproj* h, const cba_options* opts, int32_t n_sel, const int32_t* view_idx,
                                       double* cov7x7);

typedef int32_t (*cba_allreduce_fn)(double* buf, int64_t count, void* user);
cba_status cba_reproj_set_allreduce(cba_reproj* h, cba_allreduce_fn fn, void* user, int32_t n_ranks, int32_t rank);
#define CBA_RCCL_UNIQUE_ID_BYTES 128
cba_status cba_rccl_unique_id(uint8_t id[CBA_RCCL_UNIQUE_ID_BYTES]);
cba_status cba_reproj_init_rccl(cba_reproj* h, const uint8_t id[CBA_RCCL_UNIQUE_ID_BYTES],
                                int32_t n_ranks, int32_t rank);

cba_status cba_optimize_intrinsics(int32_t camera_model, int32_t n_views, const int64_t* view_offset,
                                   const double* X, const double* Y, const double* u, const double* v,
                                   double* intr, double* c_T_t , const cba_options* opts,
                                   cba_summary* summary, double* cov);
cba_status cba_optimize_extrinsics(int32_t camera_model, int32_t n_cams, int32_t n_views, int32_t n_blocks,
                                   const int64_t* blk_offset, const int32_t* blk_view, const int32_t* blk_cam,
                                   const double* X, const double* Y, const double* u, const double* v,
                                   double* intr, double* c_T_r, double* r_T_t, const cba_options* opts,
                                   cba_summary* summary, double* cov);
cba_status cba_optimize_bundle(int32_t camera_model, int32_t n_cams, int32_t n_blocks,
                               const int64_t* blk_offset, const int32_t* blk_cam, const double* blk_b_T_g,
                               const double* X, const double* Y, const double* u, const double* v,
                               double* intr, double* g_T_c, double* b_T_t, const cba_options* opts,
                               cba_summary* summary, double* cov);
cba_status cba_optimize_handeye(int32_t n_poses, const double* base_T_gripper, const double* cam_T_target,
                                double* g_T_c , const cba_options* opts, cba_summary* summary,
                                double* cov);

cba_status cba_estimate_handeye_dlt(int32_t n_poses, const double* base_T_gripper, const double* cam_T_target,
                                    double min_angle_deg, double* g_T_c );
cba_status cba_estimate_and_optimize_handeye(int32_t n_poses, const double* base_T_gripper, const double* cam_T_target,
                                             double min_angle_deg , double* g_T_c ,
                                             const cba_options* opts, cba_summary* summary, double* cov);

cba_status cba_estimate_and_optimize_handeye_sharded(int32_t n_poses, const double* base_T_gripper, const double* cam_T_target,
                                                     double min_angle_deg, int32_t estimate, double* g_T_c,
                                                     const cba_options* opts, cba_summary* summary, double* cov,
                                                     cba_allreduce_fn fn, void* user, int32_t n_ranks, int32_t rank, int32_t device);

cba_status cba_estimate_and_optimize_handeye_rccl(int32_t n_poses, const double* base_T_gripper, const double* cam_T_target,
                                                  double min_angle_deg, int32_t estimate, double* g_T_c,
                                                  const cba_options* opts, cba_summary* summary, double* cov,
                                                  const uint8_t id[CBA_RCCL_UNIQUE_ID_BYTES], int32_t n_ranks, int32_t rank,
                                                  int32_t device);

cba_status cba_optimize_planar_pose(int32_t n, const double* X, const double* Y, const double* u, const double* v,
                                    const double* kmtx5, int32_t num_radial, double* pose7, const cba_options* opts,
                                    cba_summary* summary, double* distortion, double* reprojection_error, double* cov36);
cba_status cba_optimize_planar_pose_batch(int32_t n_views, const int64_t* view_offset, const double* X, const double* Y,
                                          const double* u, const double* v, const double* kmtx5, int32_t num_radial,
                                          double* pose7, const cba_options* opts, cba_summary* summaries, double* distortion,
                                          double* reprojection_error, double* cov36);

cba_status cba_optimize_homography(int32_t n, const double* X, const double* Y, const double* u, const double* v,
                                   double* h9, const cba_options* opts, cba_summary* summary, double* cov64);
cba_status cba_optimize_homography_batch(int32_t n_views, const int64_t* view_offset, const double* X, const double* Y,
                                         const double* u, const double* v, double* h9 ,
                                         const cba_options* opts, cba_summary* summaries, double* cov64 );

cba_status cba_optimize_intrinsics_semidlt(int32_t n_views, const int64_t* view_offset, const double* X, const double* Y,
                                           const double* u, const double* v, double* kmtx5, double* c_T_t, int32_t num_radial,
                                           const double* bounds_lo5, const double* bounds_hi5, const int32_t* fixed_distortion_indices,
                                           const double* fixed_distortion_values, int32_t n_fixed, const cba_options* opts,
                                           cba_summary* summary, double* distortion, double* view_errors, double* cov);

cba_status cba_optimize_intrinsics_semidlt_sharded(int32_t n_views_local, const int64_t* view_offset, const double* X, const double* Y,
                                                   const double* u, const double* v, int32_t n_views_total, int32_t first_view,
                                                   double* kmtx5, double* c_T_t, int32_t num_radial, const double* bounds_lo5,
                                                   const double* bounds_hi5, const int32_t* fixed_distortion_indices,
                                                   const double* fixed_distortion_values, int32_t n_fixed, const cba_options* opts,
                                                   cba_summary* summary, double* distortion, double* view_errors, double* cov,
                                                   cba_allreduce_fn fn, void* user, int32_t n_ranks, int32_t rank, int32_t device);
cba_status cba_optimize_intrinsics_semidlt_rccl(int32_t n_views_local, const int64_t* view_offset, const double* X, const double* Y,
                                                const double* u, const double* v, int32_t n_views_total, int32_t first_view,
                                                double* kmtx5, double* c_T_t, int32_t num_radial, const double* bounds_lo5,
                                                const double* bounds_hi5, const int32_t* fixed_distortion_indices,
                                                const double* fixed_distortion_values, int32_t n_fixed, const cba_options* opts,
// ... 299 lines not shown
```

Baseline: 27.66 billion.

## Add narrow packed-triangle Schur path for small shared systems with controller gather

For shared-parameter systems with at most 16 unknowns, the Schur complement is accumulated as a packed upper triangle plus gradient instead of 64x64 tiles. This shrinks per-chunk partial buffers and the amount summed. A dedicated narrow syrk kernel replaces the tiled one. When the LM controller runs on a single rank, the chunk row-sum is folded into the controller kernel through LDS, which removes a separate pack launch. It can be disabled with an env var, and it adds extra code paths and LDS pressure in the controller.

```diff
diff --git a/calibration_amd/capi.py b/calibration_amd/capi.py
--- a/calibration_amd/capi.py
+++ b/calibration_amd/capi.py
@@ -293,6 +293,7 @@
     "cba_reproj_solve": (C.c_int32, [C.c_void_p, C.POINTER(CbaOptions), C.POINTER(CbaSummary)]),
     "cba_reproj_set_lm_mode": (C.c_int32, [C.c_void_p, C.c_int32]),
     "cba_reproj_solve_stats": (C.c_int32, [C.c_void_p, C.POINTER(C.c_int64)]),
+    "cba_reproj_lm_narrow": (C.c_int32, [C.c_void_p]),
     "cba_reproj_covariance_dim": (C.c_int64, [C.c_void_p]),
     "cba_reproj_covariance": (C.c_int32, [C.c_void_p, C.POINTER(CbaOptions), c_double_p]),
     "cba_reproj_covariance_shared_dim": (C.c_int64, [C.c_void_p]),
diff --git a/calibration_amd/csrc/backend_hip.hip b/calibration_amd/csrc/backend_hip.hip
--- a/calibration_amd/csrc/backend_hip.hip
+++ b/calibration_amd/csrc/backend_hip.hip
@@ -155,7 +155,11 @@
     bool vstats_pending = false;
     double ctl_huber = 0.0;
     bool can_fuse() const { return st.fuse_small && st.schur_wave && st.s.n_views != 0 && !e.scalar; }
-    void enqueue_system(double huber, bool tail, bool has_blocks, bool constrained, int which, const PackLayout& L, int has_stats, int has_cost = -1) {
+    int64_t schur_sw() const { return st.narrow ? narrow_tri(st.s.nsh) : static_cast<int64_t>(st.n_pairs) * 4096; }
+    CtlGather pending_gather{};
+    bool ctl_gathers(const PackLayout& L) const { return st.narrow && can_fuse() && L.n_ranks == 1 && !e.rccl_comm && !e.allreduce; }
+    void enqueue_system(double huber, bool tail, bool has_blocks, bool constrained, int which, const PackLayout& L, int has_stats, int has_cost = -1,
+                        bool for_ctl = false) {
         const Structure& s = st.s;
         const bool q2 = s.n_views != 0;
         if (!can_fuse()) {
@@ -165,7 +169,7 @@
             return;
         }
         const int n = s.nsh;
-        const int64_t sw = static_cast<int64_t>(st.n_pairs) * 4096;
+        const int64_t sw = schur_sw();
         if (tail && !e.head_weights)
             hipLaunchKernelGGL(k_weights, dim3(nblk(s.n_blocks, 256)), dim3(256), 0, e.stream, s.n_blocks, s.NACC, s.NH + s.PL, e.blk_acc.p,
                                huber, e.blk_w.p, e.blk_s.p);
@@ -179,6 +183,7 @@
         a.n_seg = tail ? a.n_seg_x * s.n_cams : 0;
         a.n_syrk = st.n_vchunks * st.n_pairs;
         a.has_vstats = vstats_pending ? 1 : 0;
+        a.narrow = st.narrow;
         a.huber = huber;
         a.link_off = st.link_off.p; a.cchunk_off = st.cchunk_off.p; a.cam_seg = st.cam_seg.p;
         a.link_blk = st.link_blk.p; a.cam_blk = st.cam_blk.p; a.view_fixed = e.view_fixed.p; a.view_cam_blk = st.view_cam_blk.p;
@@ -193,9 +198,17 @@
         if (n >= 64 && st.syrk_mfma) hipLaunchKernelGGL(k_sys_stage3<true>, dim3(g3), dim3(256), 0, e.stream, a);
         else hipLaunchKernelGGL(k_sys_stage3<false>, dim3(g3), dim3(256), 0, e.stream, a);
         vstats_pending = false;
-        hipLaunchKernelGGL(k_sys_pack, dim3(nblk(sw + n, RS_COLS)), dim3(RS_COLS * RS_GROUPS), 0, e.stream,
-                           pack_args(L, has_blocks, true, has_stats, has_cost), static_cast<int64_t>(st.n_vchunks), st.syrk_partial.p,
-                           st.sys_tiles.p + sw + n, st.stat_dev.p, pack_target());
+        if (for_ctl && ctl_gathers(L)) {
+            const PackArgs pa = pack_args(L, has_blocks, true, has_stats, has_cost);
+            CtlGather& G = pending_gather;
+            G.rows = st.syrk_partial.p; G.n_chunks = st.n_vchunks; G.rank = pa.rank;
+            G.has_blocks = pa.has_blocks; G.has_cost = pa.has_cost; G.has_stats = pa.has_stats;
+            G.tail = st.sys_tiles.p + sw + n; G.stat = st.stat_dev.p; G.pack = pack_target();
+        } else {
+            hipLaunchKernelGGL(k_sys_pack, dim3(nblk(sw + n, RS_COLS)), dim3(RS_COLS * RS_GROUPS), 0, e.stream,
+                               pack_args(L, has_blocks, true, has_stats, has_cost), static_cast<int64_t>(st.n_vchunks), st.syrk_partial.p,
+                               st.sys_tiles.p + sw + n, st.stat_dev.p, pack_target());
+        }
         CBA_HIP(hipGetLastError());
     }
     void collect_normal_eq(std::vector<double>& cam_acc, double cost2[2]) {
@@ -223,9 +236,13 @@
                            e.stream, st.dims, s.n_views, st.link_off.p, st.link_blk.p, e.blk_acc.p, e.blk_w.p, e.view_fixed.p, lmp_src,
                            constrained ? 1 : 0, e.view[which].p, e.view_scale2.p, e.view_L.p, e.view_y.p, e.view_D.p, e.view_gp.p, e.blk_Z.p,
                            st.view_gmax.p);
-        const int64_t sw = static_cast<int64_t>(st.n_pairs) * 4096;
-        hipLaunchKernelGGL(n >= 64 && st.syrk_mfma ? k_schur_syrk_mfma : k_schur_syrk, dim3(st.n_vchunks, st.n_pairs), dim3(256), 0, e.stream,
-                           st.dims, s.n_views, n, st.n_tiles, st.view_cam_blk.p, e.blk_Z.p, e.view_y.p, st.syrk_partial.p);
+        const int64_t sw = schur_sw();
+        if (st.narrow)
+            hipLaunchKernelGGL(k_schur_narrow, dim3(st.n_vchunks), dim3(256), 0, e.stream, st.dims, s.n_views, n, st.view_cam_blk.p, e.blk_Z.p,
+                               e.view_y.p, st.syrk_partial.p);
+        else
+            hipLaunchKernelGGL(n >= 64 && st.syrk_mfma ? k_schur_syrk_mfma : k_schur_syrk, dim3(st.n_vchunks, st.n_pairs), dim3(256), 0, e.stream,
+                               st.dims, s.n_views, n, st.n_tiles, st.view_cam_blk.p, e.blk_Z.p, e.view_y.p, st.syrk_partial.p);
         double* pack = tiles_out ? tiles_out : st.pin.p;
         hipLaunchKernelGGL(k_row_sum, dim3(nblk(sw + n, RS_COLS)), dim3(RS_COLS * RS_GROUPS), 0, e.stream, static_cast<int64_t>(st.n_vchunks),
                            sw + n, st.syrk_partial.p, pack);
@@ -235,12 +252,17 @@
     void collect_schur(std::vector<double>& S, std::vector<double>& g, double* gmax_priv, int* nfail) {
         const Structure& s = st.s;
         const int n = s.nsh;
-        const int64_t sw = static_cast<int64_t>(st.n_pairs) * 4096;
+        const int64_t sw = schur_sw();
         const double* tiles = st.pin.p;
         const int32_t nf = static_cast<int32_t>(tiles[static_cast<size_t>(sw) + n + 1] + 0.5);
         for (int i = 0; i < n; ++i) g[i] = tiles[static_cast<size_t>(sw) + i];
         *gmax_priv = tiles[static_cast<size_t>(sw) + n];
         *nfail = nf;
+        if (st.narrow) {
+            for (int i = 0; i < n; ++i)
+                for (int j = i; j < n; ++j) S[static_cast<size_t>(i) * n + j] = S[static_cast<size_t>(j) * n + i] = tiles[narrow_sidx(n, i, j)];
+            return;
+        }
         int pair = 0;
         for (int ti = 0; ti < st.n_tiles; ++ti)
             for (int tj = ti; tj < st.n_tiles; ++tj, ++pair) {
@@ -290,6 +312,7 @@
         a.off_stats = L.stats; a.off_cam = L.cam; a.off_cost = L.cost; a.off_nfail = L.nfail; a.off_S = L.S; a.off_g = L.g; a.off_gmax = L.gmax;
         a.n = s.nsh; a.n_tiles = st.n_tiles; a.n_ranks = L.n_ranks; a.rank = e.rank; a.n_cam_doubles = s.n_cams * s.NACC;
         a.has_blocks = has_blocks; a.has_schur = has_schur; a.has_stats = has_stats; a.has_cost = has_cost < 0 ? has_blocks : has_cost;
+        a.narrow = st.narrow;
         return a;
     }
     void ensure_pack(const PackLayout& L) {
@@ -475,7 +498,9 @@
         V.rec = st.ctl_rec.p;
     }
     void run_ctl(int mode, int flag) {
-        launch_lm_ctl(st.ctl_view, mode, flag, e.stream);
+        const CtlGather G = pending_gather;
+        pending_gather = CtlGather();
+        launch_lm_ctl(st.ctl_view, mode, flag, e.stream, G);
         ++ctl_invocations;
         if (st.ctl_event) {
             if (!st.ctl_done) CBA_HIP(hipEventCreateWithFlags(&st.ctl_done, hipEventDisableTiming));
@@ -518,7 +543,7 @@
         const bool q1 = s.n_blocks != 0;
         ctl_huber = huber;
         if (q1) enqueue_normal_eq_head(0, huber);
-        enqueue_system(huber, q1, q1, ctl_constrained, 0, L, 0);
+        enqueue_system(huber, q1, q1, ctl_constrained, 0, L, 0, -1, true);
         exchange(L.cam, L.size - L.cam, ar, nullptr, true);
         run_ctl(CTL_NEW, first ? 1 : 0);
         e.active = 0;
@@ -526,7 +551,7 @@
     void ctl_resolve(const PackLayout& L, const AllReduce& ar, int rank) override {
         (void)rank;
         const Structure& s = st.s;
-        enqueue_system(0.0, false, s.n_blocks != 0, ctl_constrained, 0, L, 0, 0);
+        enqueue_system(0.0, false, s.n_blocks != 0, ctl_constrained, 0, L, 0, 0, true);
         exchange(L.nfail, L.gmax - L.nfail, ar, nullptr, true);
         run_ctl(CTL_RESOLVED, 0);
     }
@@ -560,13 +585,13 @@
         }
         if (q1) with_alt_blocks([&] { enqueue_normal_eq_head(1, ctl_huber, fused_head); });
     }
-    void step_tail_enqueue(double huber, bool constrained, const PackLayout& L) {
+    void step_tail_enqueue(double huber, bool constrained, const PackLayout& L, bool for_ctl = false) {
         const Structure& s = st.s;
         const bool q1 = s.n_blocks != 0;
-        with_alt_blocks([&] { enqueue_system(huber, q1, q1, constrained, 1, L, 1); });
+        with_alt_blocks([&] { enqueue_system(huber, q1, q1, constrained, 1, L, 1, -1, for_ctl); });
     }
     void step_tail_speculative(double huber, const PackLayout& L, const AllReduce& ar) {
-        step_tail_enqueue(huber, ctl_constrained, L);
+        step_tail_enqueue(huber, ctl_constrained, L, true);
         exchange(0, L.size, ar, nullptr, true);
         run_ctl(CTL_STEP, 1);
         e.active = 1;
@@ -736,6 +761,8 @@
     st->n_vchunks = std::max(1, (s.n_views + VCHUNK - 1) / VCHUNK);
     st->n_tiles = (s.nsh + 63) / 64;
     st->n_pairs = st->n_tiles * (st->n_tiles + 1) / 2;
+    st->narrow = narrow_fits(s.nsh) ? 1 : 0;
+    if (const char* env = std::getenv("CBA_LM_NARROW")) st->narrow = st->narrow && std::atoi(env) != 0;
     std::vector<int64_t> coff{0}, cseg(s.n_cams + 1, 0);
     for (int c = 0; c < s.n_cams; ++c) {
         for (int64_t p = s.cam_off[c]; p < s.cam_off[c + 1]; p += CCHUNK) coff.push_back(std::min<int64_t>(p + CCHUNK, s.cam_off[c + 1]));
@@ -756,7 +783,8 @@
     st->view_delta.alloc(nv * 6);
     st->view_delta.zero(e.stream);
     st->view_stats.alloc(nv * 4);
-    st->syrk_partial.alloc(static_cast<size_t>(st->n_vchunks) * (static_cast<size_t>(st->n_pairs) * 4096 + s.nsh));
+    st->syrk_partial.alloc(static_cast<size_t>(st->n_vchunks) *
+                           (st->narrow ? static_cast<size_t>(narrow_width(s.nsh)) : static_cast<size_t>(st->n_pairs) * 4096 + s.nsh));
     st->pin.reserve(static_cast<size_t>(st->n_pairs) * 4096 + s.nsh + 8);
     st->pin_ne.reserve(static_cast<size_t>(s.n_cams) * s.NACC + 2);
     st->pin_tr.reserve(32);
@@ -808,6 +836,11 @@
 void solve_stats(const Engine& e, int64_t stats8[8]) {
     const HipLMState* st = reinterpret_cast<const HipLMState*>(e.lm_state);
     for (int k = 0; k < 8; ++k) stats8[k] = st ? st->xs[k] : 0;
+}
+
+int lm_narrow(const Engine& e) {
+    const HipLMState* st = reinterpret_cast<const HipLMState*>(e.lm_state);
+    return st ? st->narrow : 0;
 }
 
 void set_lm_mode(Engine& e, int mode) {
diff --git a/calibration_amd/csrc/capi.cpp b/calibration_amd/csrc/capi.cpp
--- a/calibration_amd/csrc/capi.cpp
+++ b/calibration_amd/csrc/capi.cpp
@@ -774,6 +774,8 @@
     });
 }
 
+int32_t cba_reproj_lm_narrow(const cba_reproj* h) { return h ? lm_narrow(*reinterpret_cast<const Engine*>(h)) : 0; }
+
 int64_t cba_reproj_covariance_dim(const cba_reproj* h) { return h ? covariance_dim(*reinterpret_cast<const Engine*>(h)) : 0; }
 
 cba_status cba_reproj_covariance(cba_reproj* h, const cba_options* opts, double* cov) {
diff --git a/calibration_amd/csrc/engine.hpp b/calibration_amd/csrc/engine.hpp
--- a/calibration_amd/csrc/engine.hpp
+++ b/calibration_amd/csrc/engine.hpp
@@ -126,6 +126,7 @@
 void warm_lm(Engine& e);
 void solve_lm(Engine& e, const cba_options& o, cba_summary* out);
 void solve_stats(const Engine& e, int64_t stats8[8]);
+int lm_narrow(const Engine& e);
 void set_lm_mode(Engine& e, int mode);
 void compute_covariance(Engine& e, const cba_options& o, double* cov, bool shared_only = false);
 void compute_covariance_views(Engine& e, const cba_options& o, const int32_t* views, int n_sel, double* view_cov);
diff --git a/calibration_amd/csrc/lm_core.hpp b/calibration_amd/csrc/lm_core.hpp
--- a/calibration_amd/csrc/lm_core.hpp
+++ b/calibration_amd/csrc/lm_core.hpp
@@ -311,9 +311,9 @@
                          t_queue / std::max(1, n_waits), n_head_queued, static_cast<int>(rec[CS_N_WASTED]));
         if (timing && rec[CS_PROF + CP_PUBLISH] > 0.0) {
             static const char* const names[CTL_NPROF] = {"entry", "adopt", "gradient norm", "assemble", "factorise", "back-substitute", "plus",
-                                                         "model terms", "decide", "publish", "", ""};
+                                                         "model terms", "decide", "publish", "gather", ""};
             std::fprintf(stderr, "[cba timing] controller kernel phases, us over %d invocations:", static_cast<int>(rec[CS_SEQ]));
-            for (int k = 0; k <= CP_PUBLISH; ++k) std::fprintf(stderr, " %s %.1f |", names[k], rec[CS_PROF + k] * 0.01);
+            for (int k = 0; k <= CP_GATHER; ++k) std::fprintf(stderr, " %s %.1f |", names[k], rec[CS_PROF + k] * 0.01);
             std::fprintf(stderr, "\n");
         }
         std::snprintf(out->report, sizeof(out->report), "calibba(schur LM, %d rank%s): %s iters=%d cost %.6e -> %.6e", n_ranks_,
diff --git a/calibration_amd/csrc/lm_ctl.hip b/calibration_amd/csrc/lm_ctl.hip
--- a/calibration_amd/csrc/lm_ctl.hip
+++ b/calibration_amd/csrc/lm_ctl.hip
@@ -1,5 +1,6 @@
 #include <mutex>
 #include <set>
+#include <stdexcept>
 
 #include "engine.hpp"
 #include "lm_ctl.hpp"
@@ -79,8 +80,10 @@
     }
 };
 
+__host__ __device__ inline size_t lm_ctl_lds_doubles(int n) { return static_cast<size_t>(ctl_padded(n) + 1) * ctl_lda(n); }
+
 template <bool LDS_A>
-__global__ __launch_bounds__(CTL_THREADS) void k_lm_ctl(CtlView V, int mode, int flag) {
+__global__ __launch_bounds__(CTL_THREADS) void k_lm_ctl(CtlView V, int mode, int flag, CtlGather G) {
     extern __shared__ double lds_dyn[];
     __shared__ double red[CTL_WAVES];
     __shared__ double s_Ld[LDS_A ? CTL_LDS_MAX_N * CTL_NB : 1];
@@ -120,8 +123,10 @@
     V.scal = s_scal;
     V.okflag = &s_ok;
     if (LDS_A) { V.A = lds_dyn; V.Ld = s_Ld; }
+    if (LDS_A) G.scratch = lds_dyn + lm_ctl_lds_doubles(n);
+    else G.rows = nullptr;
     __syncthreads();
-    ctl_run(tm, V, mode, flag);
+    ctl_run(tm, V, mode, flag, G);
     if (small)
         for (int i = tid; i < n; i += CTL_THREADS) {
             g_gc[i] = s_small[2 * CTL_SMALL_N + i];
@@ -132,14 +137,17 @@
         }
 }
 
-size_t lm_ctl_lds_bytes(int n) { return static_cast<size_t>(ctl_padded(n) + 1) * ctl_lda(n) * sizeof(double); }
+size_t lm_ctl_lds_bytes(int n) { return lm_ctl_lds_doubles(n) * sizeof(double); }
 bool lm_ctl_fits_lds(int n) { return n <= CTL_LDS_MAX_N; }
 
-void launch_lm_ctl(const CtlView& V, int mode, int flag, hipStream_t stream) {
+void launch_lm_ctl(const CtlView& V, int mode, int flag, hipStream_t stream, const CtlGather& G) {
+    if (G.rows && !(narrow_fits(V.n) && lm_ctl_fits_lds(V.n))) throw std::logic_error("LM controller: a chunk table to sum for a system that is not narrow");
+    static_assert(NARROW_MAX_NSH <= CTL_LDS_MAX_N, "a narrow system's controller keeps its matrix, and the group sums behind it, in LDS");
+    const size_t gather_bytes = G.rows ? sizeof(double) * NARROW_GROUPS * narrow_width(V.n) : 0;
     if (lm_ctl_fits_lds(V.n))
-        hipLaunchKernelGGL(k_lm_ctl<true>, dim3(1), dim3(CTL_THREADS), lm_ctl_lds_bytes(V.n), stream, V, mode, flag);
+        hipLaunchKernelGGL(k_lm_ctl<true>, dim3(1), dim3(CTL_THREADS), lm_ctl_lds_bytes(V.n) + gather_bytes, stream, V, mode, flag, G);
     else
-        hipLaunchKernelGGL(k_lm_ctl<false>, dim3(1), dim3(CTL_THREADS), 0, stream, V, mode, flag);
+        hipLaunchKernelGGL(k_lm_ctl<false>, dim3(1), dim3(CTL_THREADS), 0, stream, V, mode, flag, G);
     CBA_HIP(hipGetLastError());
 }
 
diff --git a/calibration_amd/csrc/lm_ctl.hpp b/calibration_amd/csrc/lm_ctl.hpp
--- a/calibration_amd/csrc/lm_ctl.hpp
+++ b/calibration_amd/csrc/lm_ctl.hpp
@@ -5,6 +5,7 @@
 #include "../../include/calibba.h"
 #include "reproj_math.hpp"
 #include "schur_math.hpp"
+#include "schur_narrow.hpp"
 
 #if defined(__HIPCC__)
 #define CBA_NOINLINE __host__ __device__ __attribute__((noinline))
@@ -34,7 +35,7 @@
     CS_COUNT = 80
 };
 constexpr int CTL_NPROF = 12;
-enum CtlProf : int { CP_ENTRY = 0, CP_ADOPT, CP_GMAX, CP_ASSEMBLE, CP_FACTOR, CP_BACKSOLVE, CP_PLUS, CP_MODEL, CP_DECIDE, CP_PUBLISH };
+enum CtlProf : int { CP_ENTRY = 0, CP_ADOPT, CP_GMAX, CP_ASSEMBLE, CP_FACTOR, CP_BACKSOLVE, CP_PLUS, CP_MODEL, CP_DECIDE, CP_PUBLISH, CP_GATHER };
 static_assert(CS_PROF + CTL_NPROF <= CS_COUNT, "control record size");
 
 enum CtlMode : int { CTL_NONE = 0, CTL_NEW = 1, CTL_RESOLVED = 2, CTL_STEP = 3, CTL_LS_DONE = 4, CTL_LINE_SEARCH = 5 };
@@ -108,6 +109,71 @@
 CBA_HD int64_t ctl_sidx(int n, int i, int j) { return i <= j ? static_cast<int64_t>(i) * n - static_cast<int64_t>(i) * (i - 1) / 2 + (j - i)
                                                               : static_cast<int64_t>(j) * n - static_cast<int64_t>(j) * (j - 1) / 2 + (i - j); }
 
+struct CtlGather {
+    const double* rows = nullptr;
+    int n_chunks = 0, rank = 0;
+    int has_blocks = 0, has_cost = 0, has_stats = 0;
+    const double* tail = nullptr;
+    const double* stat = nullptr;
+    double* pack = nullptr;
+    double* scratch = nullptr;
+};
+
+CBA_HD void ctl_pack_scalars(int64_t off_nfail, int64_t off_cost, int64_t off_stats, int has_cost, int has_stats, const double* stat,
+                             double nfail, double* pack) {
+    pack[off_nfail] = nfail;
+    pack[off_cost] = has_cost ? stat[4] : 0.0;
+    pack[off_stats + 0] = has_stats == 1 ? stat[2] : 0.0;
+    pack[off_stats + 1] = has_stats == 1 ? stat[3] : 0.0;
+    pack[off_stats + 2] = has_stats ? stat[0] : 0.0;
+    pack[off_stats + 3] = has_stats ? stat[1] : 0.0;
+    pack[off_stats + 4] = (has_stats && has_cost) ? stat[4] : 0.0;
+    pack[off_stats + 5] = has_stats == 2 ? stat[2] : 0.0;
+}
+
+template <class TM>
+CBA_HD void ctl_gather(TM& tm, const CtlView& V, const CtlGather& G) {
+    const int W = narrow_width(V.n), tri = narrow_tri(V.n);
+    constexpr int NQ = 8;
+    const int total = NARROW_GROUPS * W;
+    for (int p0 = tm.tid(); p0 < total; p0 += 2 * tm.size()) {
+        const int p1 = p0 + tm.size();
+        const bool two = p1 < total;
+        const int r0 = p0 / W, e0 = p0 - r0 * W;
+        const int r1 = two ? p1 / W : 0, e1 = two ? p1 - r1 * W : 0;
+        double s0 = 0.0, s1 = 0.0;
+        for (int b = 0; b < G.n_chunks; b += NQ * NARROW_GROUPS) {
+            double v0[NQ], v1[NQ];
+#pragma unroll
+            for (int q = 0; q < NQ; ++q) {
+                const int t0 = b + r0 + q * NARROW_GROUPS, t1 = b + r1 + q * NARROW_GROUPS;
+                v0[q] = t0 < G.n_chunks ? G.rows[static_cast<int64_t>(t0) * W + e0] : 0.0;
+                v1[q] = (two && t1 < G.n_chunks) ? G.rows[static_cast<int64_t>(t1) * W + e1] : 0.0;
+            }
+#pragma unroll
+            for (int q = 0; q < NQ; ++q)
+                if (b + r0 + q * NARROW_GROUPS < G.n_chunks) s0 += v0[q];
+#pragma unroll
+            for (int q = 0; q < NQ; ++q)
+                if (two && b + r1 + q * NARROW_GROUPS < G.n_chunks) s1 += v1[q];
+        }
+        G.scratch[p0] = s0;
+        if (two) G.scratch[p1] = s1;
+    }
+    tm.sync();
+    for (int e = tm.tid(); e < W; e += tm.size()) {
+        double tot = 0.0;
+        for (int k = 0; k < NARROW_GROUPS; ++k) tot += G.scratch[k * W + e];
+        G.pack[e < tri ? V.off_S + e : V.off_g + (e - tri)] = tot;
+    }
+    for (int r = tm.tid(); r < V.n_ranks; r += tm.size()) G.pack[V.off_gmax + r] = r == G.rank ? G.tail[0] : 0.0;
+    if (tm.tid() == 0) ctl_pack_scalars(V.off_nfail, V.off_cost, V.off_stats, G.has_cost, G.has_stats, G.stat, G.tail[1], G.pack);
+    if (!G.has_blocks)
+        for (int k = tm.tid(); k < V.n_cams * V.NACC; k += tm.size()) G.pack[V.off_cam + k] = 0.0;
+    tm.sync();
+    tm.tick(V, CP_GATHER);
+}
+
 struct CtlPlusView {
     int n_cams, PI, PC, sh_base, chain, intr_var, target_var;
     int64_t pk_cam, pk_target;
@@ -639,7 +705,8 @@
 }
 
 template <class TM>
-CBA_HD void ctl_run(TM& tm, const CtlView& V, int mode, int flag) {
+CBA_HD void ctl_run(TM& tm, const CtlView& V, int mode, int flag, const CtlGather& G = CtlGather()) {
+    if (G.rows) ctl_gather(tm, V, G);
     const bool in_turn = V.scal[CS_TERM] < 0.0 && static_cast<int>(V.scal[CS_EXPECT]) == mode &&
                          (mode != CTL_STEP || (V.scal[CS_STEP_SPEC] != 0.0) == (flag != 0));
     tm.sync();
diff --git a/calibration_amd/csrc/lm_kernels.hpp b/calibration_amd/csrc/lm_kernels.hpp
--- a/calibration_amd/csrc/lm_kernels.hpp
+++ b/calibration_amd/csrc/lm_kernels.hpp
@@ -2,6 +2,7 @@
 #include "block_reduce.hpp"
 #include "lm_ctl.hpp"
 #include "schur_math.hpp"
+#include "schur_narrow.hpp"
 #include "wave_reduce.hpp"
 
 namespace cba {
@@ -366,10 +367,53 @@
     else syrk_tile_valu(Zi, Zc, nrow, out);
     if (ti == tj) schur_gvec_chunk(Zi, ysh, nrow, i0, nsh, row + static_cast<int64_t>(gy) * 4096);
 }
+__device__ __forceinline__ void schur_narrow_body(double* lds, int bx, const SchurDims& d, int n_views, int nsh, const int32_t* __restrict__ view_cam_blk,
+        const double* __restrict__ blk_Z, const double* __restrict__ y, double* __restrict__ partial) {
+    double (*Zs)[NARROW_MAX_NSH] = reinterpret_cast<double (*)[NARROW_MAX_NSH]>(lds);
+    double* ysh = lds + SYRK_ROWS * NARROW_MAX_NSH;
+    int* bsh = reinterpret_cast<int*>(ysh + SYRK_ROWS);
+    const int v0 = bx * VCHUNK;
+    const int nrow = 6 * (min(n_views, v0 + VCHUNK) - v0);
+    const bool table = d.n_cams <= SYRK_MAX_CAMS;
+    stage_block_table(d, n_views, v0, view_cam_blk, bsh);
+    __syncthreads();
+    for (int idx = threadIdx.x; idx < SYRK_ROWS * NARROW_MAX_NSH; idx += 256) {
+        const int row = idx / NARROW_MAX_NSH, g = idx % NARROW_MAX_NSH;
+        const int gg = g < nsh ? g : 0;
+        const int cam = gg / d.PC, lc = gg - cam * d.PC;
+        const int v = v0 + row / 6;
+        const int b = table ? bsh[(row / 6) * d.n_cams + cam] : (v < n_views ? view_cam_blk[static_cast<int64_t>(v) * d.n_cams + cam] : -1);
+        const double z = blk_Z[(static_cast<int64_t>(b < 0 ? 0 : b) * 6 + row % 6) * d.PSH + lc];
+        Zs[row][g] = (g < nsh && b >= 0) ? z : 0.0;
+    }
+    if (static_cast<int>(threadIdx.x) < SYRK_ROWS) ysh[threadIdx.x] = static_cast<int>(threadIdx.x) < nrow ? y[6 * static_cast<int64_t>(v0) + threadIdx.x] : 0.0;
+    __syncthreads();
+    const int e = threadIdx.x, tri = narrow_tri(nsh);
+    if (e >= tri + nsh) return;
+    double s = 0.0;
+    if (e < tri) {
+        int i, j;
+        narrow_ij(nsh, e, &i, &j);
+        for (int r = 0; r < nrow; ++r) s += Zs[r][i] * Zs[r][j];
+    } else {
+        const int c = e - tri;
+        for (int r = 0; r < nrow; ++r) s += Zs[r][c] * ysh[r];
+    }
+    partial[static_cast<int64_t>(bx) * (tri + nsh) + e] = s;
+}
+static_assert(NARROW_GROUPS == RS_GROUPS, "the controller sums the chunk rows in grouped_column_sum's order");
+static_assert(NARROW_MAX_WIDTH <= 256, "one thread per entry of the narrow row");
+static_assert(SYRK_ROWS * NARROW_MAX_NSH + SYRK_ROWS + VCHUNK * SYRK_MAX_CAMS / 2 <= SYRK_LDS, "the narrow body lives in the syrk bodies' LDS");
+
 __global__ __launch_bounds__(256) void k_schur_syrk(SchurDims d, int n_views, int nsh, int n_tiles, const int32_t* __restrict__ view_cam_blk,
         const double* __restrict__ blk_Z, const double* __restrict__ y, double* __restrict__ partial) {
     __shared__ double lds[SYRK_LDS];
     schur_syrk_body<false>(lds, blockIdx.x, blockIdx.y, gridDim.y, d, n_views, nsh, n_tiles, view_cam_blk, blk_Z, y, partial);
+}
+__global__ __launch_bounds__(256) void k_schur_narrow(SchurDims d, int n_views, int nsh, const int32_t* __restrict__ view_cam_blk,
+        const double* __restrict__ blk_Z, const double* __restrict__ y, double* __restrict__ partial) {
+    __shared__ double lds[SYRK_LDS];
+    schur_narrow_body(lds, blockIdx.x, d, n_views, nsh, view_cam_blk, blk_Z, y, partial);
 }
 __global__ __launch_bounds__(256) void k_schur_syrk_mfma(SchurDims d, int n_views, int nsh, int n_tiles, const int32_t* __restrict__ view_cam_blk,
         const double* __restrict__ blk_Z, const double* __restrict__ y, double* __restrict__ partial) {
@@ -405,27 +449,24 @@
     int64_t off_stats, off_cam, off_cost, off_nfail, off_S, off_g, off_gmax;
     int n, n_tiles, n_ranks, rank, n_cam_doubles;
     int has_blocks , has_cost , has_schur, has_stats;
+    int narrow;
 };
 __device__ __forceinline__ void pack_scalars(const PackArgs& a, const double* __restrict__ stat, double nfail, double* __restrict__ pack) {
-    pack[a.off_nfail] = nfail;
-    pack[a.off_cost] = a.has_cost ? stat[4] : 0.0;
-    pack[a.off_stats + 0] = a.has_stats == 1 ? stat[2] : 0.0;
-    pack[a.off_stats + 1] = a.has_stats == 1 ? stat[3] : 0.0;
-    pack[a.off_stats + 2] = a.has_stats ? stat[0] : 0.0;
-    pack[a.off_stats + 3] = a.has_stats ? stat[1] : 0.0;
-    pack[a.off_stats + 4] = (a.has_stats && a.has_cost) ? stat[4] : 0.0;
-    pack[a.off_stats + 5] = a.has_stats == 2 ? stat[2] : 0.0;
+    ctl_pack_scalars(a.off_nfail, a.off_cost, a.off_stats, a.has_cost, a.has_stats, stat, nfail, pack);
 }
 __global__ __launch_bounds__(256) void k_pack(PackArgs a, const double* __restrict__ stat ,
-                                              const double* __restrict__ tiles , double* __restrict__ pack) {
+                                              const double* __restrict__ tiles ,
+                                              double* __restrict__ pack) {
     const int64_t tid = static_cast<int64_t>(blockIdx.x) * blockDim.x + threadIdx.x;
     const int64_t nn = static_cast<int64_t>(a.n) * a.n;
-    const int64_t sw = static_cast<int64_t>(a.n_tiles) * (a.n_tiles + 1) / 2 * 4096;
+    const int64_t sw = a.narrow ? narrow_tri(a.n) : static_cast<int64_t>(a.n_tiles) * (a.n_tiles + 1) / 2 * 4096;
     if (tid < nn) {
         const int i = static_cast<int>(tid / a.n), j = static_cast<int>(tid % a.n);
         if (i <= j) {
             double val = 0.0;
-            if (a.has_schur) {
+            if (a.has_schur && a.narrow) {
+                val = tiles[narrow_sidx(a.n, i, j)];
+            } else if (a.has_schur) {
                 const int ti = i >> 6, tj = j >> 6;
                 const int pair = ti * a.n_tiles - ti * (ti - 1) / 2 + (tj - ti);
                 val = tiles[static_cast<int64_t>(pair) * 4096 + (i & 63) * 64 + (j & 63)];
@@ -445,6 +486,7 @@
     int n_cc, n_vb, n_costp;
     int n_seg_x, n_seg, n_syrk;
     int has_vstats;
+    int narrow;
     double huber;
     const int64_t *link_off, *cchunk_off, *cam_seg;
     const int32_t *link_blk, *cam_blk, *view_fixed, *view_cam_blk;
@@ -483,7 +525,8 @@
     bx -= a.n_seg;
     if (bx < a.n_syrk) {
         const int chunk = bx % a.n_vchunks, pair = bx / a.n_vchunks;
-        schur_syrk_body<MFMA>(lds, chunk, pair, a.n_pairs, a.d, a.n_views, a.nsh, a.n_tiles, a.view_cam_blk, a.blk_Z, a.view_y, a.syrk_partial);
+        if (a.narrow) schur_narrow_body(lds, chunk, a.d, a.n_views, a.nsh, a.view_cam_blk, a.blk_Z, a.view_y, a.syrk_partial);
+        else schur_syrk_body<MFMA>(lds, chunk, pair, a.n_pairs, a.d, a.n_views, a.nsh, a.n_tiles, a.view_cam_blk, a.blk_Z, a.view_y, a.syrk_partial);
         return;
     }
     bx -= a.n_syrk;
@@ -501,11 +544,13 @@
                                                                    const double* __restrict__ tail ,
                                                                    const double* __restrict__ stat, double* __restrict__ pack) {
     __shared__ double sh[RS_GROUPS][RS_COLS];
-    const int64_t sw = static_cast<int64_t>(a.n_tiles) * (a.n_tiles + 1) / 2 * 4096, width = sw + a.n;
+    const int64_t sw = a.narrow ? narrow_tri(a.n) : static_cast<int64_t>(a.n_tiles) * (a.n_tiles + 1) / 2 * 4096, width = sw + a.n;
     const int64_t e = static_cast<int64_t>(blockIdx.x) * RS_COLS + threadIdx.x % RS_COLS;
     const double tot = grouped_column_sum(rows, 0, n_rows, width, e, e < width, sh);
     if (threadIdx.x < RS_COLS && e < width) {
-        if (e < sw) {
+        if (e < sw && a.narrow) {
+            pack[a.off_S + e] = tot;
+        } else if (e < sw) {
             int ti, tj;
             tile_pair(static_cast<int>(e >> 12), a.n_tiles, &ti, &tj);
             const int i = ti * 64 + static_cast<int>((e >> 6) & 63), j = tj * 64 + static_cast<int>(e & 63);
diff --git a/calibration_amd/csrc/lm_state.hpp b/calibration_amd/csrc/lm_state.hpp
--- a/calibration_amd/csrc/lm_state.hpp
+++ b/calibration_amd/csrc/lm_state.hpp
@@ -13,6 +13,7 @@
     int fuse_small = 1;
     int schur_wave = 1;
     int syrk_mfma = 1;
+    int narrow = 0;
     DevBuf<int32_t> view_cam_blk, cam_blk;
     DevBuf<int64_t> cchunk_off, cam_seg, link_off;
     DevBuf<int32_t> link_blk;
@@ -68,7 +69,7 @@
 void resident_lm_warm(Engine& e);
 bool resident_lm_solve(Engine& e, const cba_options& o, cba_summary* out, bool keep_parameters = false);
 
-void launch_lm_ctl(const CtlView& V, int mode, int flag, hipStream_t stream);
+void launch_lm_ctl(const CtlView& V, int mode, int flag, hipStream_t stream, const CtlGather& G = CtlGather());
 bool lm_ctl_fits_lds(int n);
 void warm_lm_ctl();
 
diff --git a/calibration_amd/csrc/schur_narrow.hpp b/calibration_amd/csrc/schur_narrow.hpp
--- /dev/null
+++ b/calibration_amd/csrc/schur_narrow.hpp
@@ -0,0 +1,23 @@
+#pragma once
+#include <cstdint>
+
+namespace cba {
+
+constexpr int NARROW_MAX_NSH = 16;
+
+constexpr bool narrow_fits(int n) { return n >= 1 && n <= NARROW_MAX_NSH; }
+constexpr int narrow_tri(int n) { return n * (n + 1) / 2; }
+constexpr int narrow_width(int n) { return narrow_tri(n) + n; }
+constexpr int NARROW_MAX_WIDTH = narrow_width(NARROW_MAX_NSH);
+constexpr int NARROW_GROUPS = 8;
+
+constexpr int narrow_sidx(int n, int i, int j) { return i <= j ? i * n - i * (i - 1) / 2 + (j - i) : j * n - j * (j - 1) / 2 + (i - j); }
+constexpr int narrow_gidx(int n, int i) { return narrow_tri(n) + i; }
+constexpr void narrow_ij(int n, int e, int* i, int* j) {
+    int r = 0;
+    while (e >= n - r) { e -= n - r; ++r; }
+    *i = r;
+    *j = r + e;
+}
+
+}
diff --git a/calibration_amd/optim.py b/calibration_amd/optim.py
--- a/calibration_amd/optim.py
+++ b/calibration_amd/optim.py
@@ -393,6 +393,9 @@
 
     def set_lm_mode(self, mode: int):
         capi.check(self.lib, self.lib.cba_reproj_set_lm_mode(self.h, int(mode)))
+
+    def lm_narrow(self) -> bool:
+        return bool(self.lib.cba_reproj_lm_narrow(self.h))
 
     def solve_stats(self) -> dict:
         a = (C.c_int64 * 8)()
diff --git a/include/calibba.h b/include/calibba.h
--- a/include/calibba.h
+++ b/include/calibba.h
@@ -127,6 +127,8 @@
 cba_status cba_reproj_set_lm_mode(cba_reproj* h, int32_t mode);
 
 cba_status cba_reproj_solve_stats(const cba_reproj* h, int64_t stats8[8]);
+
+int32_t cba_reproj_lm_narrow(const cba_reproj* h);
 
 int64_t cba_reproj_covariance_dim(const cba_reproj* h);
 cba_status cba_reproj_covariance(cba_reproj* h, const cba_options* opts, double* cov );
```

Measured after the change: 27.63 billion. No clear change (-0.1%).
